# uthree/ALiVE-VC

Measured on AMD Instinct MI355X. Metric: VC frames/sec + RTF @24kHz, 1M-vec library; 1/2/4/8 MI355X, higher is better.
Workload: dtype decoder fp16 GEMMs / fp32 acc; encoders 22-bit fp16 split; kNN exact fp32 top-k via fp6 MFMA candidates (certified); f32 MFMA small convs; f64 phase scan

## Files before the change

### alive-vc_amd/csrc/knn.hip

```cpp
#include "common.h"

namespace {

constexpr int D = ALIVE_DIM;
constexpr int KP = ALIVE_KPRIME;
constexpr int TILE = 128;
constexpr int MAX_SPLIT = 64;

__device__ __forceinline__ float wave_sum(float v) {
#pragma unroll
    for (int o = 32; o > 0; o >>= 1) v += __shfl_xor(v, o);
    return v;
}

struct NormDiv {
    float n, y;
};
__device__ __forceinline__ NormDiv norm_div(float n) {
    float y = __builtin_amdgcn_rcpf(n);
    const float e = fmaf(-n, y, 1.0f);
    y = fmaf(e, y, y);
    return NormDiv{n, y};
}
__device__ __forceinline__ float div_by(float x, const NormDiv& d) {
// ... 339 lines not shown
    for (int i = 0; i < D / 256; ++i) xs[tid + 256 * i] = v[i];
    __syncthreads();
    if (tid < 4) {
        for (int d = tid; d < D; d += 4) ss = fmaf(xs[d], xs[d], ss);
        red[tid] = ss;
    }
    __syncthreads();
    const float nrm = sqrtf(red[0] + red[1] + red[2] + red[3]);
    if (nrm_out != nullptr && tid == 0) nrm_out[ft] = nrm;
    float e2 = 0.0f;
#pragma unroll
    for (int i = 0; i < D / 256; ++i) {
        const float q = nrm > 0.0f ? v[i] / nrm : 0.0f;
        s_f32[(size_t)ft * D + tid + 256 * i] = q;
        const unsigned short b = f32_to_bf16_rn(q);
        s_bf16[(size_t)ft * D + tid + 256 * i] = b;
        const float e = q - __uint_as_float((unsigned)b << 16);
        e2 = fmaf(e, e, e2);
    }
    if (dq != nullptr) {
        e2 = wave_sum(e2);
        if ((tid & 63) == 0) ered[tid >> 6] = e2;
        __syncthreads();
        if (tid == 0) dq[ft] = sqrtf(ered[0] + ered[1] + ered[2] + ered[3]) * 1.0001f;
    }
}

constexpr int KH = KP / 2;
constexpr int FT = 256;
constexpr int LT = 32;
constexpr int NK16 = D / 16;
constexpr int PIECE = 1152;
constexpr int NPIECE = 4 * (D / 64);
constexpr int ABUF = NPIECE * PIECE;
constexpr int SCORE_LDS = 2 * ABUF + FT * KP * 8;

constexpr int GATE_BOOL = -2;
__device__ __forceinline__ bool gate_open(const int* cnt, int lo, int hi, int& c) {
    c = 0x7fffffff;
    if (cnt == nullptr) return true;
    c = *cnt;
    return c > lo && c <= hi;
}

__global__ __launch_bounds__(128) void gather_frames_kernel(const unsigned short* __restrict__ s_bf16, const int* __restrict__ list,
                                                            const int* __restrict__ cnt, int lo, int hi, unsigned short* __restrict__ out) {
    int c;
    if (!gate_open(cnt, lo, hi, c)) return;
    const int slot = blockIdx.x;
    if (slot >= (c + 255) / 256 * 256) return;
    if (threadIdx.x >= 96) return;
    u32x4 v = {0u, 0u, 0u, 0u};
    if (slot < c) v = ((const u32x4*)(s_bf16 + (size_t)list[slot] * D))[threadIdx.x];
    ((u32x4*)(out + (size_t)slot * D))[threadIdx.x] = v;
}

typedef const __attribute__((address_space(1))) void* gptr_t;
typedef __attribute__((address_space(3))) void* lptr_t;

struct SeedArgs {
    float* tau;
    int* flag;
    int k;
    float margin;
    int* cnt;
};

__device__ __forceinline__ bool seeds_look(const SeedArgs& sa, int split) {
    __shared__ int verdict[1];
    if (sa.tau == nullptr || split == 0) return false;
    if (threadIdx.x == 0) {
        const int f = __hip_atomic_load(sa.flag + (size_t)(split - 1) * gridDim.x + blockIdx.x, __ATOMIC_RELAXED, __HIP_MEMORY_SCOPE_AGENT);
        if (f != 0) {
            atomicAdd(sa.cnt, 1);
            __builtin_amdgcn_fence(__ATOMIC_ACQUIRE, "agent");
        }
        verdict[0] = f;
    }
    asm volatile("s_waitcnt vmcnt(0)" ::: "memory");
    __syncthreads();
    return __builtin_amdgcn_readfirstlane(verdict[0]) != 0;
}

template <int KH_, int WF_ = 64, int FRAMES_ = 256>
__device__ __forceinline__ void seeds_publish(const SeedArgs& sa, const float* Lv, const int* Li, int64_t frame0, int split, bool seeded) {
    constexpr int LW_ = 4 * 2 * WF_;
    for (int col = threadIdx.x; col < FRAMES_; col += 256) {
        const int lcb = (col / WF_) * (2 * WF_) + ((col % WF_) >> 5) * 64 + (col & 31);
        float prev = INFINITY;
        for (int j = 0; j < sa.k; ++j) {
            float m = -INFINITY;
            for (int e = 0; e < 2 * KH_; ++e) {
                const int o = (e % KH_) * LW_ + lcb + (e / KH_) * 32;
                const float v = Lv[o];
                if (Li[o] >= 0 && v < prev) m = fmaxf(m, v);
            }
            prev = m;
        }
        float t = prev - sa.margin;
        if (seeded) {
            const float tin = sa.tau[frame0 + col];
            t = fmaxf(t, tin == tin ? tin : -INFINITY);
        }
        sa.tau[frame0 + col] = t;
    }
    asm volatile("s_waitcnt vmcnt(0)" ::: "memory");
    __syncthreads();
    if (threadIdx.x == 0) {
        __builtin_amdgcn_fence(__ATOMIC_RELEASE, "agent");
        asm volatile("s_waitcnt vmcnt(0)" ::: "memory");
        __hip_atomic_store(sa.flag + (size_t)split * gridDim.x + blockIdx.x, 1, __ATOMIC_RELAXED, __HIP_MEMORY_SCOPE_AGENT);
    }
}

struct PoolBlocks {
    const int* hdr;
    const int* blk_voice;
    const int64_t* img_off;
    const int32_t* seg_lo;
    const int32_t* seg_len;
};
enum { PH_GROUPS = 0, PH_BLOCKS, PH_ITEMS, PH_FAIL, PH_WORDS = 8 };

template <bool COLLECT, bool POOL = false>
__global__ __launch_bounds__(256, 1) void knn_score_kernel(const unsigned short* __restrict__ s_bf16,
                                                           const unsigned short* __restrict__ lib, int64_t M, int tiles_total,
                                                           int tiles_per_split, int P, float* __restrict__ cand_val,
                                                           int* __restrict__ cand_idx, const int* __restrict__ gate_cnt,
                                                           int gate_lo, int gate_hi, int by_count, const float* __restrict__ thr_in,
                                                           SeedArgs sa, int caps, PoolBlocks pool = PoolBlocks{}) {
    int n_slots = 0x7fffffff;
    {
        int c;
        if (!gate_open(gate_cnt, gate_lo, gate_hi, c)) return;
        if (by_count && (int64_t)blockIdx.x * 256 >= c) return;
        if (by_count) n_slots = c;
    }
    int row_base = 0;
    if constexpr (POOL) {
        if ((int)blockIdx.x >= pool.hdr[PH_BLOCKS]) return;
        const int v = pool.blk_voice[blockIdx.x];
        M = pool.seg_len[v];
        lib += (size_t)pool.img_off[v] * D;
        tiles_total = (int)(((M + TILE - 1) / TILE * TILE) / LT);
        tiles_per_split = (tiles_total + (int)gridDim.y - 1) / (int)gridDim.y;
        row_base = pool.seg_lo[v];
    }
    extern __shared__ __attribute__((aligned(16))) unsigned char smem[];
    float* Lv = (float*)(smem + 2 * ABUF);
    int* Li = (int*)(Lv + FT * KP);

    const int tid = threadIdx.x, lane = tid & 63;
    const int w = __builtin_amdgcn_readfirstlane(tid >> 6);
    const int lr = lane & 31, lh = lane >> 5;
    const int64_t frame0 = (int64_t)blockIdx.x * FT;
    const int split = blockIdx.y;
    const int tile_begin = split * tiles_per_split;
    int tile_end = tile_begin + tiles_per_split;
    if (tile_end > tiles_total) tile_end = tiles_total;

    const bool seeded = !COLLECT && seeds_look(sa, split);
    float seed[2] = {-INFINITY, -INFINITY};
    if (seeded) {
#pragma unroll
        for (int ni = 0; ni < 2; ++ni) {
            const float t = sa.tau[frame0 + 64 * w + 32 * ni + lr];
            seed[ni] = t == t ? t : -INFINITY;
        }
    }
    int* cntF = (int*)Lv;
    if (COLLECT) {
        cntF[tid] = 0;
        for (int e = tid; e < FT * caps; e += 256) {
            const size_t o = ((size_t)(frame0 + e / caps) * P + split) * caps + e % caps;
            cand_val[o] = -INFINITY;
            cand_idx[o] = -1;
        }
    } else {
// ... 275 lines not shown
            bf16x8 a[PD + 1];
#pragma unroll
            for (int i = 0; i < PD; ++i) a[i] = *(const bf16x8*)(Ab + a_off[i & 3] + (i >> 2) * 4 * PIECE);
#pragma unroll
            for (int ks = 0; ks < NK16; ++ks) {
                if (ks + PD < NK16) a[(ks + PD) % (PD + 1)] = *(const bf16x8*)(Ab + a_off[(ks + PD) & 3] + ((ks + PD) >> 2) * 4 * PIECE);
                if ((ks & 3) == 1)
                    __builtin_amdgcn_global_load_lds((gptr_t)(gnext + (ks >> 2) * 64), (lptr_t)(lnext + (ks >> 2) * 4 * PIECE), 16, 0, 0);
                __builtin_amdgcn_sched_barrier(0);
                acc = __builtin_amdgcn_mfma_f32_32x32x16_bf16(a[ks % (PD + 1)], bq[0][ks], acc, 0, 0, 0);
                __builtin_amdgcn_sched_barrier(0);
            }
        }
        const int64_t row0 = (int64_t)tile * LT;
        const bool ragged = row0 + LT > M;
        float mx = -INFINITY;
#pragma unroll
        for (int r = 0; r < 16; ++r) {
            if (ragged && row0 + (r & 3) + 8 * (r >> 2) + 4 * lh >= M) acc[r] = -INFINITY;
            mx = fmaxf(mx, acc[r]);
        }
        while (__builtin_amdgcn_ballot_w64(mx >= thr && mx > -INFINITY) != 0) {
            const bool has = mx >= thr && mx > -INFINITY;
            int rsel = 0;
#pragma unroll
            for (int r = 1; r < 16; ++r) rsel = (acc[r] == mx) ? r : rsel;
            if (has) {
                const int pos = atomicAdd(&cntF[32 * w + lr], 1);
                if (pos < caps) {
                    cand_val[seg + pos] = mx;
                    cand_idx[seg + pos] = (int)(row0 + (rsel & 3) + 8 * (rsel >> 2) + 4 * lh);
                }
            }
            float nmx = -INFINITY;
#pragma unroll
            for (int r = 0; r < 16; ++r) {
                if (has && r == rsel) acc[r] = -INFINITY;
                nmx = fmaxf(nmx, acc[r]);
            }
            mx = nmx;
        }
        __syncthreads();
    }
    if (tid < FT2 && cntF[tid] > caps) cand_idx[((size_t)(frame0 + tid) * P + split) * caps] = -2;
}

constexpr int KH8 = 16;
constexpr int KP8 = 2 * KH8;
constexpr int NK64 = D / 64;
constexpr int NPIECE8 = 4 * (D / 128);
constexpr int ABUF8 = NPIECE8 * PIECE;
constexpr int FT6 = 4 * 32 * 3;
constexpr int SCORE8_LDS = 2 * ABUF8 + FT * KP8 * 8;
constexpr int SCORE6_LDS = 2 * ABUF8 + FT6 * KP8 * 8;
typedef int v8i __attribute__((ext_vector_type(8)));

constexpr float SEED_MARGIN8 = 0.02f * F8_SCALE * F8_SCALE;
constexpr float SEED_MARGIN6 = 0.024f * F6_SCALE * F6_SCALE;
constexpr float SEED_MARGIN16 = 2.5e-3f;
constexpr float SEED_MARGIN16_STRICT = 4.5e-3f;
constexpr int SEED_MIN_FB = 512;
constexpr int SEED_MIN_FB6 = 300;

template <int FMT, int NCT8, int NK = NK64>
__device__ __forceinline__ void knn_score8_body(const unsigned char* __restrict__ s_f8,
                                                const unsigned char* __restrict__ lib, int64_t M, int tiles_total,
                                                int tiles_per_split, int P, float* __restrict__ cand_val,
                                                int* __restrict__ cand_idx, const int* __restrict__ gate_cnt,
                                                int gate_lo, int gate_hi, SeedArgs sa,
                                                const float* __restrict__ rho = nullptr, const float* __restrict__ gq = nullptr) {
    {
        int c;
        if (!gate_open(gate_cnt, gate_lo, gate_hi, c)) return;
    }
    constexpr int WF8 = 32 * NCT8;
    constexpr int FT8 = 4 * WF8;
    constexpr int LW8 = 4 * 2 * WF8;
    constexpr int KD = 64 * NK;
    constexpr int NSEG = KD / 128;
    constexpr int ABUF_ = 4 * NSEG * PIECE;
    extern __shared__ __attribute__((aligned(16))) unsigned char smem[];
    float* Lv = (float*)(smem + 2 * ABUF_);
    int* Li = (int*)(Lv + FT8 * KP8);

    const int tid = threadIdx.x, lane = tid & 63;
    const int w = __builtin_amdgcn_readfirstlane(tid >> 6);
    const int lr = lane & 31, lh = lane >> 5;
    const int64_t frame0 = (int64_t)blockIdx.x * FT8;
    const int split = blockIdx.y;
    const int tile_begin = split * tiles_per_split;
    int tile_end = tile_begin + tiles_per_split;
    if (tile_end > tiles_total) tile_end = tiles_total;

    const bool seeded = seeds_look(sa, split);
    float seed[NCT8];
#pragma unroll
    for (int ni = 0; ni < NCT8; ++ni) seed[ni] = -INFINITY;
    if (seeded) {
#pragma unroll
        for (int ni = 0; ni < NCT8; ++ni) {
            const float t = sa.tau[frame0 + WF8 * w + 32 * ni + lr];
            seed[ni] = t == t ? t : -INFINITY;
        }
    }
#pragma unroll
    for (int ni = 0; ni < NCT8; ++ni)
#pragma unroll
        for (int q = 0; q < KH8; ++q) { Lv[q * LW8 + w * (2 * WF8) + ni * 64 + lane] = seed[ni]; Li[q * LW8 + w * (2 * WF8) + ni * 64 + lane] = -1; }

    const int dma_row = 8 * w + (lane >> 3);
    const int dma_chunk = (lane & 7) ^ (lane >> 3);
    auto issue_tile = [&](int tile, int buf) {
        const unsigned char* g = lib + ((size_t)tile * LT + dma_row) * KD + dma_chunk * 16;
        unsigned char* l = smem + buf * ABUF_ + w * PIECE;
#pragma unroll
        for (int sg = 0; sg < NSEG; ++sg)
            __builtin_amdgcn_global_load_lds((gptr_t)(g + sg * 128), (lptr_t)(l + sg * 4 * PIECE), 16, 0, 0);
    };
    if (tile_begin < tile_end) issue_tile(tile_begin, 0);

    v8i bq[NCT8][NK];
#pragma unroll
    for (int ni = 0; ni < NCT8; ++ni) {
        const unsigned char* fp = s_f8 + (size_t)(frame0 + WF8 * w + 32 * ni + lr) * KD + 32 * lh;
#pragma unroll
        for (int ks = 0; ks < NK; ++ks) {
            if constexpr (FMT == 2) {
                const u32x4 lo = *(const u32x4*)(fp + 64 * ks);
                const uint2 hi = *(const uint2*)(fp + 64 * ks + 16);
                bq[ni][ks] = v8i{(int)lo[0], (int)lo[1], (int)lo[2], (int)lo[3], (int)hi.x, (int)hi.y, 0, 0};
            } else {
                const u32x4 lo = *(const u32x4*)(fp + 64 * ks), hi = *(const u32x4*)(fp + 64 * ks + 16);
                bq[ni][ks] = v8i{(int)lo[0], (int)lo[1], (int)lo[2], (int)lo[3], (int)hi[0], (int)hi[1], (int)hi[2], (int)hi[3]};
            }
        }
    }

    float gs[NCT8];
#pragma unroll
    for (int ni = 0; ni < NCT8; ++ni) gs[ni] = NK == NK64 ? 0.0f : gq[frame0 + WF8 * w + 32 * ni + lr] * (F6_SCALE * F6_SCALE);

    const int rr = lr & 7;
    int a_off[2][2];
#pragma unroll
    for (int j = 0; j < 2; ++j)
#pragma unroll
        for (int c = 0; c < 2; ++c) a_off[j][c] = (lr >> 3) * PIECE + rr * 128 + (((4 * j + 2 * lh + c) ^ rr) << 4);

    float qv[NCT8][4];
    int qp[NCT8][4];
#pragma unroll
    for (int ni = 0; ni < NCT8; ++ni)
#pragma unroll
        for (int q = 0; q < 4; ++q) { qv[ni][q] = seed[ni]; qp[ni][q] = 4 * q; }
    float thr[NCT8];
#pragma unroll
    for (int ni = 0; ni < NCT8; ++ni) thr[ni] = seed[ni];
    const int lc0 = w * (2 * WF8) + lane;
    __syncthreads();

    auto load_a = [&](const unsigned char* Ab, int ks) {
        const unsigned char* q = Ab + (ks >> 1) * 4 * PIECE;
        if constexpr (FMT == 2) {
            unsigned off0 = (unsigned)(uintptr_t)(lptr_t)(q + a_off[ks & 1][0]);
            const unsigned off1 = (unsigned)(uintptr_t)(lptr_t)(q + a_off[ks & 1][1]);
            uint2 h8;
            asm volatile("ds_read_b64 %0, %2" : "=v"(h8), "+v"(off0) : "v"(off1));
            const u32x4 lo = *(const __attribute__((address_space(3))) u32x4*)(uintptr_t)off0;
            return v8i{(int)lo[0], (int)lo[1], (int)lo[2], (int)lo[3], (int)h8.x, (int)h8.y, 0, 0};
        }
        const u32x4 lo = *(const u32x4*)(q + a_off[ks & 1][0]);
        const u32x4 hi = *(const u32x4*)(q + a_off[ks & 1][1]);
        return v8i{(int)lo[0], (int)lo[1], (int)lo[2], (int)lo[3], (int)hi[0], (int)hi[1], (int)hi[2], (int)hi[3]};
    };

    auto mask_ragged = [&](f32x16& acc, int tile) {
        const int64_t row0 = (int64_t)tile * LT;
        if (row0 + LT > M) {
            asm volatile("" ::: "memory");
            const int left = (int)(M - row0);
#pragma unroll
            for (int r = 0; r < 16; ++r)
                if (4 * lh >= left - ((r & 3) + 8 * (r >> 2))) acc[r] = -INFINITY;
        }
    };
    auto max8 = [&](const f32x16& acc, int lo, float m) {
#pragma unroll
        for (int r = 0; r < 8; ++r) m = fmaxf(m, acc[lo + r]);
        return m;
    };
    auto load_rho = [&](int tile, float* rv) {
#pragma unroll
        for (int j = 0; j < 4; ++j) {
            const f32x4 t = *(const f32x4*)(rho + (size_t)tile * LT + 8 * j + 4 * lh);
#pragma unroll
            for (int e = 0; e < 4; ++e) rv[4 * j + e] = t[e];
        }
    };
    auto max8g = [&](f32x16& acc, int lo, float m, int ni, const float* rv) {
#pragma unroll
        for (int r = 0; r < 8; ++r) acc[lo + r] = fmaf(gs[ni], rv[lo + r], acc[lo + r]);
        return max8(acc, lo, m);
    };
    auto fold_loop = [&](f32x16& acc, int ni, int tile, float mx) {
        const int64_t row0 = (int64_t)tile * LT;
        float* lv = Lv + lc0 + ni * 64;
        int* li = Li + lc0 + ni * 64;
        while (__builtin_amdgcn_ballot_w64(mx > thr[ni]) != 0) {
            const bool has = mx > thr[ni];
            const bool b01 = qv[ni][1] < qv[ni][0], b23 = qv[ni][3] < qv[ni][2];
            const float m01 = b01 ? qv[ni][1] : qv[ni][0], m23 = b23 ? qv[ni][3] : qv[ni][2];
            const int p01 = b01 ? qp[ni][1] : qp[ni][0], p23 = b23 ? qp[ni][3] : qp[ni][2];
            const bool bq = m23 < m01;
            const int tpos = bq ? p23 : p01;
            const int tq = tpos >> 2;
            if (has) {
                lv[tpos * LW8] = mx;
                li[tpos * LW8] = (int)(row0 + ((__float_as_uint(mx) & 3u) + 8u * ((__float_as_uint(mx) >> 2) & 3u)) + 4 * lh);
            }
            const float* qb = lv + (tq * 4) * LW8;
            const float x0 = qb[0], x1 = qb[LW8], x2 = qb[2 * LW8], x3 = qb[3 * LW8];
            const bool c1 = x1 < x0, c3 = x3 < x2;
            const float n01 = c1 ? x1 : x0, n23 = c3 ? x3 : x2;
            const int e01 = c1 ? 1 : 0, e23 = c3 ? 3 : 2;
            const bool c = n23 < n01;
            const float nq = c ? n23 : n01;
            const int np = tq * 4 + (c ? e23 : e01);
#pragma unroll
            for (int q = 0; q < 4; ++q) {
                const bool hit = has && tq == q;
                qv[ni][q] = hit ? nq : qv[ni][q];
                qp[ni][q] = hit ? np : qp[ni][q];
            }
            thr[ni] = fminf(fminf(qv[ni][0], qv[ni][1]), fminf(qv[ni][2], qv[ni][3]));
            float nmx = -INFINITY;
#pragma unroll
            for (int r = 0; r < 16; ++r) nmx = fmaxf(nmx, acc[r] < mx ? acc[r] : -INFINITY);
            mx = has ? nmx : mx;
        }
    };

    auto fold_rare = [&](f32x16& acc, int ni, int tile, float mx) {
        if (__builtin_amdgcn_ballot_w64(mx > thr[ni]) == 0) return;
        const int64_t row0 = (int64_t)tile * LT;
        float* lv = Lv + lc0 + ni * 64;
        int* li = Li + lc0 + ni * 64;
        const bool b01 = qv[ni][1] < qv[ni][0], b23 = qv[ni][3] < qv[ni][2];
        const float m01 = b01 ? qv[ni][1] : qv[ni][0], m23 = b23 ? qv[ni][3] : qv[ni][2];
        const int p01 = b01 ? qp[ni][1] : qp[ni][0], p23 = b23 ? qp[ni][3] : qp[ni][2];
        const int tpos = m23 < m01 ? p23 : p01;
        const int tq = tpos >> 2, te = tpos & 3;
        const float* qb = lv + (tq * 4) * LW8;
        float x0 = qb[0], x1 = qb[LW8], x2 = qb[2 * LW8], x3 = qb[3 * LW8];
#pragma unroll
        for (int r = 0; r < 16; ++r) acc[r] = __uint_as_float((__float_as_uint(acc[r]) & ~15u) | (unsigned)r);
        if (row0 + LT > M) {
            asm volatile("" ::: "memory");
            const int left = (int)(M - row0);
#pragma unroll
            for (int r = 0; r < 16; ++r)
                if (4 * lh >= left - ((r & 3) + 8 * (r >> 2))) acc[r] = -INFINITY;
        }
        float m1 = -INFINITY, m2 = -INFINITY;
#pragma unroll
        for (int r = 0; r < 16; ++r) {
            m2 = __builtin_amdgcn_fmed3f(m1, m2, acc[r]);
            m1 = fmaxf(m1, acc[r]);
        }
        const bool has = m1 > thr[ni];
        if (has) {
            const unsigned u = __float_as_uint(m1);
            lv[tpos * LW8] = m1;
            li[tpos * LW8] = (int)(row0 + ((u & 3u) + 8u * ((u >> 2) & 3u)) + 4 * lh);
        }
        x0 = (has && te == 0) ? m1 : x0;
        x1 = (has && te == 1) ? m1 : x1;
        x2 = (has && te == 2) ? m1 : x2;
        x3 = (has && te == 3) ? m1 : x3;
        const bool c1 = x1 < x0, c3 = x3 < x2;
        const float n01 = c1 ? x1 : x0, n23 = c3 ? x3 : x2;
        const int e01 = c1 ? 1 : 0, e23 = c3 ? 3 : 2;
        const bool c = n23 < n01;
        const float nq = c ? n23 : n01;
        const int np = tq * 4 + (c ? e23 : e01);
#pragma unroll
        for (int q = 0; q < 4; ++q) {
            const bool hit = has && tq == q;
            qv[ni][q] = hit ? nq : qv[ni][q];
            qp[ni][q] = hit ? np : qp[ni][q];
        }
        thr[ni] = fminf(fminf(qv[ni][0], qv[ni][1]), fminf(qv[ni][2], qv[ni][3]));
        fold_loop(acc, ni, tile, m2);
    };
    if constexpr (NCT8 == 3) {
    auto do_tile3 = [&](int tile, f32x16& c0, f32x16& c1, f32x16& c2, f32x16& p0, f32x16& p1, f32x16& p2, float* rv, float* rn) {
        const int buf = (tile - tile_begin) & 1;
        const int next_tile = tile + 1 < tile_end ? tile + 1 : tile;
        const unsigned char* gnext = lib + ((size_t)next_tile * LT + dma_row) * KD + dma_chunk * 16;
        unsigned char* lnext = smem + (buf ^ 1) * ABUF_ + w * PIECE;
        const unsigned char* Ab = smem + buf * ABUF_;
#pragma unroll
        for (int r = 0; r < 16; ++r) { c0[r] = 0.0f; c1[r] = 0.0f; c2[r] = 0.0f; }
        if constexpr (NK != NK64) load_rho(tile, rn);
        constexpr int PD6 = 1, NA6 = PD6 + 1;
        v8i a[NA6];
#pragma unroll
        for (int i = 0; i < PD6; ++i) a[i] = load_a(Ab, i);
        float pm0 = -INFINITY, pm1 = -INFINITY, pm2 = -INFINITY;
        ALIVE_CHAIN_GAP(7);
#define K8_STEP3(ks, AFTER0, AFTER1, AFTER2)                                                                                     \
        {                                                                                                                        \
            __builtin_amdgcn_sched_barrier(0);                                                                                   \
            c0 = __builtin_amdgcn_mfma_scale_f32_32x32x64_f8f6f4(a[(ks) % NA6], bq[0][ks], c0, FMT, FMT, 0, 127, 0, 127); \
            __builtin_amdgcn_sched_barrier(0);                                                                                   \
            if ((ks) + PD6 < NK) a[((ks) + PD6) % NA6] = load_a(Ab, (ks) + PD6);                                                 \
            if ((ks) < NSEG)                                                                                                     \
                __builtin_amdgcn_global_load_lds((gptr_t)(gnext + (ks) * 128), (lptr_t)(lnext + (ks) * 4 * PIECE), 16, 0, 0);    \
            AFTER0;                                                                                                              \
            __builtin_amdgcn_sched_barrier(0);                                                                                   \
            c1 = __builtin_amdgcn_mfma_scale_f32_32x32x64_f8f6f4(a[(ks) % NA6], bq[1][ks], c1, FMT, FMT, 0, 127, 0, 127); \
            __builtin_amdgcn_sched_barrier(0);                                                                                   \
            AFTER1;                                                                                                              \
            __builtin_amdgcn_sched_barrier(0);                                                                                   \
            c2 = __builtin_amdgcn_mfma_scale_f32_32x32x64_f8f6f4(a[(ks) % NA6], bq[2][ks], c2, FMT, FMT, 0, 127, 0, 127); \
            __builtin_amdgcn_sched_barrier(0);                                                                                   \
            AFTER2;                                                                                                              \
        }
        f32x16 v0, v1, v2;
        auto acc_read = [&](const f32x16& a_, int lo, int hi, f32x16& v) {
#pragma unroll
            for (int r = lo; r < hi; ++r) asm volatile("v_accvgpr_read_b32 %0, %1" : "=v"(v[r]) : "a"(a_[r]));
        };
        auto acc_pin = [&]() { asm volatile("" : "+a"(c0), "+a"(c1), "+a"(c2)); };
        K8_STEP3(0, (void)0, (void)0, (void)0) K8_STEP3(1, (void)0, (void)0, (void)0) K8_STEP3(2, (void)0, (void)0, (void)0)
        if constexpr (NK == NK64) {
        K8_STEP3(3, (void)0, (void)0, (void)0) K8_STEP3(4, (void)0, (void)0, (void)0) K8_STEP3(5, (void)0, (void)0, acc_pin())
        }
        if constexpr (NK == NK64) {
        K8_STEP3(6, acc_read(p0, 0, 8, v0), (acc_pin(), acc_read(p0, 8, 16, v0), mask_ragged(v0, tile - 1)), (acc_pin(), pm0 = max8(v0, 0, pm0)))
        K8_STEP3(7, pm0 = max8(v0, 8, pm0), fold_rare(v0, 0, tile - 1, pm0), (acc_pin(), acc_read(p1, 0, 8, v1)))
        K8_STEP3(8, (acc_pin(), acc_read(p1, 8, 16, v1), mask_ragged(v1, tile - 1)), (acc_pin(), pm1 = max8(v1, 0, pm1)), pm1 = max8(v1, 8, pm1))
        K8_STEP3(9, fold_rare(v1, 1, tile - 1, pm1), (acc_pin(), acc_read(p2, 0, 8, v2)), (acc_pin(), acc_read(p2, 8, 16, v2), mask_ragged(v2, tile - 1)))
        K8_STEP3(10, (acc_pin(), pm2 = max8(v2, 0, pm2)), pm2 = max8(v2, 8, pm2), fold_rare(v2, 2, tile - 1, pm2))
        K8_STEP3(11, (void)0, (void)0, (void)0)
        } else {
        K8_STEP3(3, acc_pin(), (acc_pin(), acc_read(p0, 0, 8, v0)), (acc_pin(), acc_read(p0, 8, 16, v0), mask_ragged(v0, tile - 1)))
        K8_STEP3(4, (acc_pin(), pm0 = max8g(v0, 0, pm0, 0, rv)), pm0 = max8g(v0, 8, pm0, 0, rv), fold_rare(v0, 0, tile - 1, pm0))
        K8_STEP3(5, (acc_pin(), acc_read(p1, 0, 8, v1)), (acc_pin(), acc_read(p1, 8, 16, v1), mask_ragged(v1, tile - 1)), (acc_pin(), pm1 = max8g(v1, 0, pm1, 1, rv)))
        K8_STEP3(6, pm1 = max8g(v1, 8, pm1, 1, rv), fold_rare(v1, 1, tile - 1, pm1), (acc_pin(), acc_read(p2, 0, 8, v2)))
        K8_STEP3(7, (acc_pin(), acc_read(p2, 8, 16, v2), mask_ragged(v2, tile - 1)), (acc_pin(), pm2 = max8g(v2, 0, pm2, 2, rv)),
                 (pm2 = max8g(v2, 8, pm2, 2, rv), fold_rare(v2, 2, tile - 1, pm2)))
        }
#undef K8_STEP3
        acc_pin();
        __syncthreads();
    };
    auto fold_now3 = [&](f32x16& p0, f32x16& p1, f32x16& p2, int tile, float* rv) {
        mask_ragged(p0, tile);
        mask_ragged(p1, tile);
        mask_ragged(p2, tile);
        if constexpr (NK != NK64) {
            (void)max8g(p0, 0, max8g(p0, 8, -INFINITY, 0, rv), 0, rv);
            (void)max8g(p1, 0, max8g(p1, 8, -INFINITY, 1, rv), 1, rv);
            (void)max8g(p2, 0, max8g(p2, 8, -INFINITY, 2, rv), 2, rv);
        }
        fold_rare(p0, 0, tile, max8(p0, 8, max8(p0, 0, -INFINITY)));
        fold_rare(p1, 1, tile, max8(p1, 8, max8(p1, 0, -INFINITY)));
        fold_rare(p2, 2, tile, max8(p2, 8, max8(p2, 0, -INFINITY)));
    };
    {
        f32x16 A0, A1, A2, B0, B1, B2;
        float RA[16], RB[16];
#pragma unroll
        for (int r = 0; r < 16; ++r) { B0[r] = -INFINITY; B1[r] = -INFINITY; B2[r] = -INFINITY; RA[r] = 0.0f; RB[r] = 0.0f; }
        int tile = tile_begin;
        for (; tile + 1 < tile_end; tile += 2) {
            do_tile3(tile, A0, A1, A2, B0, B1, B2, RB, RA);
            do_tile3(tile + 1, B0, B1, B2, A0, A1, A2, RA, RB);
        }
        if (tile < tile_end) {
            do_tile3(tile, A0, A1, A2, B0, B1, B2, RB, RA);
            fold_now3(A0, A1, A2, tile, RA);
        } else if (tile_begin < tile_end) {
            fold_now3(B0, B1, B2, tile_end - 1, RB);
        }
    }
    } else {
    auto do_tile = [&](int tile, f32x16& c0, f32x16& c1, f32x16& p0, f32x16& p1) {
        const int buf = (tile - tile_begin) & 1;
        const int next_tile = tile + 1 < tile_end ? tile + 1 : tile;
        const unsigned char* gnext = lib + ((size_t)next_tile * LT + dma_row) * KD + dma_chunk * 16;
        unsigned char* lnext = smem + (buf ^ 1) * ABUF_ + w * PIECE;
        const unsigned char* Ab = smem + buf * ABUF_;
#pragma unroll
        for (int r = 0; r < 16; ++r) { c0[r] = 0.0f; c1[r] = 0.0f; }
        v8i a[2];
        a[0] = load_a(Ab, 0);
        float pm0 = -INFINITY, pm1 = -INFINITY;
#ifndef ALIVE_KNN8_NO_CHAIN_GAP
        ALIVE_CHAIN_GAP(7);
#endif
#define K8_STEP(ks, AFTER0, AFTER1)                                                                                              \
        {                                                                                                                        \
            __builtin_amdgcn_sched_barrier(0);                                                                                   \
            c0 = __builtin_amdgcn_mfma_scale_f32_32x32x64_f8f6f4(a[(ks) & 1], bq[0][ks], c0, FMT, FMT, 0, 127, 0, 127);              \
            __builtin_amdgcn_sched_barrier(0);                                                                                   \
            if ((ks) + 1 < NK) a[((ks) + 1) & 1] = load_a(Ab, (ks) + 1);                                                         \
            if ((ks) < NSEG)      \
                                 \
                __builtin_amdgcn_global_load_lds((gptr_t)(gnext + (ks) * 128), (lptr_t)(lnext + (ks) * 4 * PIECE), 16, 0, 0);    \
            AFTER0;                                                                                                              \
            __builtin_amdgcn_sched_barrier(0);                                                                                   \
            c1 = __builtin_amdgcn_mfma_scale_f32_32x32x64_f8f6f4(a[(ks) & 1], bq[1][ks], c1, FMT, FMT, 0, 127, 0, 127);              \
            __builtin_amdgcn_sched_barrier(0);                                                                                   \
            AFTER1;                                                                                                              \
        }
        f32x16 v0, v1;
        auto acc_read = [&](const f32x16& a, int lo, int hi, f32x16& v) {
#pragma unroll
            for (int r = lo; r < hi; ++r) asm volatile("v_accvgpr_read_b32 %0, %1" : "=v"(v[r]) : "a"(a[r]));
        };
        auto acc_pin = [&]() { asm volatile("" : "+a"(c0), "+a"(c1)); };
        K8_STEP(0, (void)0, (void)0) K8_STEP(1, (void)0, (void)0) K8_STEP(2, (void)0, (void)0) K8_STEP(3, (void)0, (void)0)
        K8_STEP(4, (void)0, (void)0) K8_STEP(5, (void)0, acc_pin())
        K8_STEP(6, acc_read(p0, 0, 8, v0), (acc_pin(), acc_read(p0, 8, 16, v0), mask_ragged(v0, tile - 1)))
        K8_STEP(7, (acc_pin(), pm0 = max8(v0, 0, pm0)), pm0 = max8(v0, 8, pm0))
        K8_STEP(8, (acc_pin(), acc_read(p1, 0, 8, v1)), (acc_pin(), acc_read(p1, 8, 16, v1), mask_ragged(v1, tile - 1)))
        K8_STEP(9, (acc_pin(), pm1 = max8(v1, 0, pm1)), pm1 = max8(v1, 8, pm1))
        K8_STEP(10, (void)0, fold_rare(v0, 0, tile - 1, pm0))
        K8_STEP(11, (void)0, fold_rare(v1, 1, tile - 1, pm1))
#undef K8_STEP
        asm volatile("" : "+a"(c0), "+a"(c1));
        __syncthreads();
    };
    auto fold_now = [&](f32x16& p0, f32x16& p1, int tile) {
        mask_ragged(p0, tile);
        mask_ragged(p1, tile);
        fold_rare(p0, 0, tile, max8(p0, 8, max8(p0, 0, -INFINITY)));
        fold_rare(p1, 1, tile, max8(p1, 8, max8(p1, 0, -INFINITY)));
    };

    f32x16 A0, A1, B0, B1;
#pragma unroll
    for (int r = 0; r < 16; ++r) { B0[r] = -INFINITY; B1[r] = -INFINITY; }
    int tile = tile_begin;
    for (; tile + 1 < tile_end; tile += 2) {
        do_tile(tile, A0, A1, B0, B1);
        do_tile(tile + 1, B0, B1, A0, A1);
    }
    if (tile < tile_end) {
        do_tile(tile, A0, A1, B0, B1);
        fold_now(A0, A1, tile);
    } else if (tile_begin < tile_end) {
        fold_now(B0, B1, tile_end - 1);
    }
    }
    __syncthreads();

    for (int e = tid; e < FT8 * KP8; e += 256) {
        const int k = e % KP8, col = e / KP8;
        const int lc = (col / WF8) * (2 * WF8) + ((col % WF8) >> 5) * 64 + (k / KH8) * 32 + (col & 31);
        const size_t o = (((size_t)(frame0 + col)) * P + split) * KP8 + k;
        cand_val[o] = Lv[(k % KH8) * LW8 + lc];
        cand_idx[o] = Li[(k % KH8) * LW8 + lc];
    }
    if (sa.tau != nullptr) seeds_publish<KH8, WF8, FT8>(sa, Lv, Li, frame0, split, seeded);
}

__global__ __launch_bounds__(256, 1) void knn_score8_kernel(const unsigned char* __restrict__ s_f8, const unsigned char* __restrict__ lib,
                                                            int64_t M, int tiles_total, int tiles_per_split, int P,
                                                            float* __restrict__ cand_val, int* __restrict__ cand_idx,
                                                            const int* __restrict__ gate_cnt, int gate_lo, int gate_hi, SeedArgs sa) {
    knn_score8_body<0, 2>(s_f8, lib, M, tiles_total, tiles_per_split, P, cand_val, cand_idx, gate_cnt, gate_lo, gate_hi, sa);
}
__global__ __launch_bounds__(256, 1) void knn_probe8_kernel(const unsigned char* __restrict__ s_f8, const unsigned char* __restrict__ lib,
                                                            int64_t M, int tiles_total, int tiles_per_split, int P,
                                                            float* __restrict__ cand_val, int* __restrict__ cand_idx, const int* __restrict__ gate) {
    knn_score8_body<0, 2>(s_f8, lib, M, tiles_total, tiles_per_split, P, cand_val, cand_idx, gate, 0, 1, SeedArgs{nullptr, nullptr, 0, 0.0f, nullptr});
}
__global__ __launch_bounds__(256, 1) void knn_score6_kernel(const unsigned char* __restrict__ s_f6, const unsigned char* __restrict__ lib,
                                                            int64_t M, int tiles_total, int tiles_per_split, int P,
                                                            float* __restrict__ cand_val, int* __restrict__ cand_idx,
                                                            const int* __restrict__ gate_cnt, int gate_lo, int gate_hi, SeedArgs sa) {
    knn_score8_body<2, 3>(s_f6, lib, M, tiles_total, tiles_per_split, P, cand_val, cand_idx, gate_cnt, gate_lo, gate_hi, sa);
}
__global__ __launch_bounds__(256, 1) void knn_probe6_kernel(const unsigned char* __restrict__ s_f6, const unsigned char* __restrict__ lib,
                                                            int64_t M, int tiles_total, int tiles_per_split, int P,
                                                            float* __restrict__ cand_val, int* __restrict__ cand_idx, const int* __restrict__ gate) {
    knn_score8_body<2, 3>(s_f6, lib, M, tiles_total, tiles_per_split, P, cand_val, cand_idx, gate, 0, 1, SeedArgs{nullptr, nullptr, 0, 0.0f, nullptr});
}
constexpr int NK_SUB = 8;
constexpr int SUB_K = 64 * NK_SUB;
constexpr int SUB6_LDS = 2 * 4 * (SUB_K / 128) * PIECE + FT6 * KP8 * 8;
__global__ __launch_bounds__(256, 1) void knn_sub6_kernel(const unsigned char* __restrict__ s_sub, const unsigned char* __restrict__ lib_sub,
                                                          const float* __restrict__ rho, const float* __restrict__ gq,
                                                          int64_t M, int tiles_total, int tiles_per_split, int P,
                                                          float* __restrict__ cand_val, int* __restrict__ cand_idx,
                                                          const int* __restrict__ gate_cnt, int gate_lo, int gate_hi, SeedArgs sa) {
    knn_score8_body<2, 3, NK_SUB>(s_sub, lib_sub, M, tiles_total, tiles_per_split, P, cand_val, cand_idx, gate_cnt, gate_lo, gate_hi, sa,
                                  rho, gq);
}

template <int G>
__device__ __forceinline__ float wave_sum_frames(float (&d)[G], int lane) {
    if constexpr (G >= 16) {
        const bool up = lane & 32;
#pragma unroll
        for (int j = 0; j < 8; ++j) d[j] = (up ? d[8 + j] : d[j]) + __shfl_xor(up ? d[j] : d[8 + j], 32);
    }
    if constexpr (G >= 8) {
        constexpr int o = G >= 16 ? 16 : 32;
        const bool up = lane & o;
#pragma unroll
        for (int j = 0; j < 4; ++j) d[j] = (up ? d[4 + j] : d[j]) + __shfl_xor(up ? d[j] : d[4 + j], o);
    }
    if constexpr (G >= 4) {
        constexpr int o = G >= 16 ? 8 : (G >= 8 ? 16 : 32);
        const bool up = lane & o;
#pragma unroll
        for (int j = 0; j < 2; ++j) d[j] = (up ? d[2 + j] : d[j]) + __shfl_xor(up ? d[j] : d[2 + j], o);
    }
    if constexpr (G >= 2) {
        constexpr int o = G >= 16 ? 4 : (G >= 8 ? 8 : (G >= 4 ? 16 : 32));
        const bool up = lane & o;
        d[0] = (up ? d[1] : d[0]) + __shfl_xor(up ? d[0] : d[1], o);
    }
    float v = d[0];
#pragma unroll
    for (int o = 32 / G; o > 0; o >>= 1) v += __shfl_xor(v, o);
    return v;
}

__device__ __forceinline__ int wave_argbest(float v, int idx) {
    float bv = v;
    int bi = idx;
    int bl = threadIdx.x & 63;
#pragma unroll
    for (int o = 32; o > 0; o >>= 1) {
        float ov = __shfl_xor(bv, o);
        int oi = __shfl_xor(bi, o);
        int ol = __shfl_xor(bl, o);
        bool take = (ov > bv) || (ov == bv && (unsigned)oi < (unsigned)bi) || (ov == bv && oi == bi && ol < bl);
        if (take) { bv = ov; bi = oi; bl = ol; }
    }
    return bl;
}

struct PoolRescore {
    const int* slot_grp;
    const int* grp;
    int* gfail;
    int* fb;
};
enum { PG_VOICE = 0, PG_MSTART, PG_SIZE, PG_BLK0, PG_NBLK, PG_CHUNKS, PG_NSLAB, PG_BASE, PG_FBASE, PG_K, PG_FIELDS };

template <int PER, bool POOL = false, bool HAT = false>
__global__ __launch_bounds__(256) __attribute__((amdgpu_waves_per_eu(HAT && PER < 16 ? 8 : 1))) void knn_rescore_kernel(const float* __restrict__ cand_val, const int* __restrict__ cand_idx,
                                                          int P, int kp, const float* __restrict__ s_f32,
                                                          const float* __restrict__ rows, const float* __restrict__ norms,
                                                          const float* __restrict__ rows_hat,
                                                          int64_t Tt, int64_t idx_base, int k, float* __restrict__ out_val,
                                                          int* __restrict__ out_idx, const int* __restrict__ frame_list,
                                                          const int* __restrict__ gate_cnt, int gate_lo, int gate_hi,
                                                          int* __restrict__ flag_list, int* __restrict__ flag_cnt, float zsig,
                                                          int list_len, float pre_scale, float sd_prior,
                                                          const float* __restrict__ det_q, const float* __restrict__ det_lib,
                                                          float* __restrict__ thr_list, int collect, float overflow_slack,
                                                          const unsigned char* __restrict__ force_fail = nullptr,
                                                          PoolRescore pool = PoolRescore{}) {
    __shared__ float cs_v[4][64];
    __shared__ int cs_i[4][64];
    const int lane = threadIdx.x & 63, wv = threadIdx.x >> 6;
    const int64_t slot = (int64_t)blockIdx.x * 4 + wv;
    int gc;
    if (gate_lo == GATE_BOOL) {
        if (*gate_cnt == 0) return;
        gc = 0x7fffffff;
    } else if (!gate_open(gate_cnt, gate_lo, gate_hi, gc)) {
        return;
    }
    if (slot >= Tt || (frame_list != nullptr && slot >= gc)) return;
    const int64_t ft = frame_list != nullptr ? frame_list[slot] : slot;
// ... 897 lines not shown
            const float up_v = __shfl_up(lv, 1);
            const int up_i = __shfl_up(li, 1);
            const bool up_before = (lane % k == 0) ? true : (up_v > p || (up_v == p && up_i < (int)r));
            if (live && !before) {
                lv = up_before ? p : up_v;
                li = up_before ? (int)r : up_i;
            }
            if (G < 16) {
                q0 = n0; q1 = n1; q2 = n2; nn = nnn;
            } else if (r + nw < M) {
                const f32x4* rp = (const f32x4*)(rows + (size_t)(r + nw) * D);
                q0 = rp[lane]; q1 = rp[lane + 64]; q2 = rp[lane + 128];
                nn = norms[r + nw];
            }
        }
        part_val[(size_t)item * 64 + lane] = lv;
        part_idx[(size_t)item * 64 + lane] = li;
    }
}

template <int G>
__global__ __launch_bounds__(256) void knn_exact_merge_kernel(const float* __restrict__ part_val, const int* __restrict__ part_idx,
                                                              int64_t Tt, int k, int64_t idx_base, const int* __restrict__ frame_list,
                                                              const int* __restrict__ cnt_ptr, float* __restrict__ out_val,
                                                              int* __restrict__ out_idx, int max_count) {
    __shared__ float sv[256];
    __shared__ int si[256], sw[256];
    const int tid = threadIdx.x;
    int64_t count = Tt;
    if (cnt_ptr != nullptr) { const int c = *cnt_ptr; count = c < Tt ? c : Tt; }
    if (count > max_count) return;
    const int64_t groups = (count + G - 1) / G;
    const int nw = exact_nw(groups);
    constexpr int NL = EX_NW_MAX / 256;
    for (int64_t slot = blockIdx.x; slot < count; slot += gridDim.x) {
        const int64_t g = slot / G;
        const int t = (int)(slot - g * G);
        const int64_t ft = frame_list != nullptr ? frame_list[slot] : slot;
        int head[NL];
#pragma unroll
        for (int i = 0; i < NL; ++i) head[i] = 0;
        for (int j = 0; j < k; ++j) {
            float bv = -INFINITY;
            int bi = 0x7fffffff, bl = -1;
#pragma unroll
            for (int i = 0; i < NL; ++i) {
                const int w = tid + 256 * i;
                if (w < nw && head[i] < k) {
                    const size_t o = ((size_t)g * nw + w) * 64 + t * k + head[i];
                    const float v = part_val[o];
                    const int id = part_idx[o];
                    if (v > bv || (v == bv && id < bi)) { bv = v; bi = id; bl = i; }
                }
            }
            sv[tid] = bv; si[tid] = bi; sw[tid] = tid;
            __syncthreads();
            for (int o = 128; o > 0; o >>= 1) {
                if (tid < o) {
                    const float ov = sv[tid + o];
                    const int oi = si[tid + o];
                    if (ov > sv[tid] || (ov == sv[tid] && oi < si[tid])) { sv[tid] = ov; si[tid] = oi; sw[tid] = sw[tid + o]; }
                }
                __syncthreads();
            }
            if (tid == 0) {
                out_val[(size_t)ft * k + j] = sv[0];
                out_idx[(size_t)ft * k + j] = (si[0] == 0x7fffffff || !(sv[0] > -INFINITY)) ? -1 : (int)(idx_base + si[0]);
            }
            if (sw[0] == tid && bl >= 0) {
#pragma unroll
                for (int i = 0; i < NL; ++i)
                    if (i == bl) head[i]++;
            }
            __syncthreads();
        }
    }
}

constexpr int COLLECT_MIN = 256;
constexpr int RESEARCH_MIN = 64;
enum { ST_FLAG8 = 0, ST_FLAG16 = 1, ST_PROBE_N = 2, ST_PROBE_FAIL = 3, ST_MODE = 4, ST_FIRST = 5, ST_PROBE_CNT = 6, ST_TIER = 7, ST_FLAGC = 8, ST_SEEDED = 9, ST_SEEDED16 = 10, ST_RESEARCH_MIN = 11, ST_COLLECT_MIN = 12,
       ST_PROBE_SKIPPED = 13,
       ST_SUB_FLAG = 14, ST_SUB_CLIP = 15, ST_SUB_FORM = 20, ST_SUB_GATE = 21,
       ST_HIST_TAG = 16, ST_HIST_STREAK = 17, ST_HIST_CALLS = 18, ST_PROBE_GATE = 19,
       ST_WORDS = 32 };
constexpr int PROBE_EVERY = 16, PROBE_STREAK = 2;
enum { TIER_SCAN = 1, TIER_EXACT_ALL = 2, TIER_BF16 = 3, TIER_FP8 = 4, TIER_FP6 = 5 };
__device__ __forceinline__ bool fp6_slot(const float* v, u32x4* o) {
    unsigned long long acc = 0;
    int nb = 0, wi = 0;
    unsigned wd[6];
    bool clipped = false;
#pragma unroll
    for (int j = 0; j < 32; ++j) {
        clipped = clipped || fabsf(v[j]) > 7.75f;
        acc |= (unsigned long long)fp6_e2m3(v[j]) << nb;
        nb += 6;
        if (nb >= 32) { wd[wi++] = (unsigned)acc; acc >>= 32; nb -= 32; }
    }
    o[0] = u32x4{wd[0], wd[1], wd[2], wd[3]};
    o[1] = u32x4{wd[4], wd[5], 0u, 0u};
    return clipped;
}
constexpr int SUB_C = 576;
__global__ __launch_bounds__(256) void lib_sub6_kernel(const float* __restrict__ y, int64_t count, int64_t span, unsigned char* __restrict__ out,
                                                       float* __restrict__ rho, int* __restrict__ clip) {
    const int64_t i = (int64_t)blockIdx.x * 256 + threadIdx.x;
    if (i >= span * (SUB_K / 32)) return;
    const int64_t r = i / (SUB_K / 32);
    const int grp = (int)(i % (SUB_K / 32));
    float v[32];
#pragma unroll
    for (int j = 0; j < 32; ++j) v[j] = r < count ? y[(size_t)r * SUB_C + 32 * grp + j] * F6_SCALE : 0.0f;
    if (fp6_slot(v, (u32x4*)(out + (size_t)r * SUB_K + 32 * grp))) atomicOr(clip, 1);
    if (grp == 0) rho[r] = r < count ? y[(size_t)r * SUB_C + SUB_K] : 0.0f;
}
constexpr float SUB_RES2 = 1.0e-5f;
__global__ __launch_bounds__(256) void sub_codes_kernel(const float* __restrict__ y, const float* __restrict__ nrm, int T, int64_t Tt,
                                                        int64_t Tt_pad, unsigned char* __restrict__ out, float* __restrict__ g,
                                                        unsigned char* __restrict__ flag, int* __restrict__ stats) {
    __shared__ float ssq[8][32];
    __shared__ int clp[8][32];
    const int fl = threadIdx.x & 31, cg = threadIdx.x >> 5;
    const int64_t f = (int64_t)blockIdx.x * 32 + fl;
    const bool live = f < Tt;
    const int64_t ni = live ? f / T : 0, ti = live ? f - ni * T : 0;
    const float* yb = y + (size_t)ni * SUB_C * T + ti;
    const float q = live ? nrm[f] : 0.0f;
    const float inv = q > 0.0f ? 1.0f / q : 0.0f;
    float v[32];
    float sy = 0.0f;
    bool clipped = false;
#pragma unroll
    for (int h = 0; h < 2; ++h) {
#pragma unroll
        for (int j = 0; j < 32; ++j) {
            v[j] = live ? yb[(size_t)(32 * (cg + 8 * h) + j) * T] * inv : 0.0f;
            sy = fmaf(v[j], v[j], sy);
            v[j] *= F6_SCALE;
        }
        u32x4 o[2];
        clipped = fp6_slot(v, o) || clipped;
        if (f < Tt_pad) {
            u32x4* dst = (u32x4*)(out + (size_t)f * SUB_K + 32 * (cg + 8 * h));
            dst[0] = o[0];
            dst[1] = o[1];
        }
    }
    const float gy = live ? yb[(size_t)SUB_K * T] * inv : 0.0f;
    if (cg == 0) sy = fmaf(gy, gy, sy);
    ssq[cg][fl] = sy;
    clp[cg][fl] = clipped ? 1 : 0;
    __syncthreads();
    if (cg == 0 && f < Tt_pad) {
        float s2 = 0.0f;
        int cl = 0;
#pragma unroll
        for (int k = 0; k < 8; ++k) { s2 += ssq[k][fl]; cl |= clp[k][fl]; }
        const bool out_of_span = q > 0.0f && 1.0f - s2 > SUB_RES2;
        const bool bad = live && (cl != 0 || out_of_span);
        g[f] = gy;
        flag[f] = bad ? 1 : 0;
        if (bad) atomicAdd(stats + ST_SUB_FLAG, 1);
        if (live && cl != 0) atomicAdd(stats + ST_SUB_CLIP, 1);
    }
}
__global__ __launch_bounds__(256) void sub_select_kernel(const unsigned char* __restrict__ flag, unsigned char* __restrict__ clip6,
                                                         int64_t n, int* __restrict__ stats) {
    const bool sub = stats[ST_SUB_FLAG] <= RESEARCH_MIN;
    const int64_t i = (int64_t)blockIdx.x * 256 + threadIdx.x;
    if (sub && i < n && flag[i] != 0) clip6[i] = 1;
    if (i == 0) {
        stats[ST_SUB_FORM] = sub ? 1 : 2;
        stats[ST_SUB_GATE] = stats[ST_MODE] != 0 ? 0 : (sub ? 1 : 2);
    }
}

__global__ void stats_init_kernel(int* __restrict__ stats, int tier, int hist_tag = 0) {
    if (threadIdx.x < ST_HIST_TAG)
        stats[threadIdx.x] = threadIdx.x == ST_TIER ? tier
                           : threadIdx.x == ST_RESEARCH_MIN ? RESEARCH_MIN : threadIdx.x == ST_COLLECT_MIN ? COLLECT_MIN : 0;
    if (threadIdx.x == ST_HIST_TAG) {
        const bool valid = hist_tag != 0 && stats[ST_HIST_TAG] == hist_tag;
        const int streak = valid ? stats[ST_HIST_STREAK] : 0, calls = valid ? stats[ST_HIST_CALLS] : 0;
        const bool skip = streak >= PROBE_STREAK && (calls % PROBE_EVERY) != 0;
        stats[ST_HIST_TAG] = hist_tag;
        stats[ST_HIST_STREAK] = streak;
        stats[ST_HIST_CALLS] = calls + 1;
        stats[ST_PROBE_GATE] = skip ? 0 : 1;
        stats[ST_PROBE_SKIPPED] = skip ? 1 : 0;
    }
}
__global__ void probe_history_kernel(int* __restrict__ stats, int64_t Tt) {
    const bool clean = stats[ST_MODE] == 0 && (int64_t)stats[ST_FLAG8] * 20 <= Tt &&
                       (stats[ST_PROBE_GATE] == 0 || (int64_t)stats[ST_PROBE_FAIL] * 4 <= (int64_t)stats[ST_PROBE_N]);
    stats[ST_HIST_STREAK] = clean ? stats[ST_HIST_STREAK] + 1 : 0;
}
__global__ __launch_bounds__(64) void probe_gather_kernel(const unsigned char* __restrict__ s_f8, int64_t Tt, int n, int n_pad,
                                                          unsigned char* __restrict__ out, int* __restrict__ plist, const int* __restrict__ gate) {
    if (*gate == 0) return;
    const int slot = blockIdx.x;
    if (slot >= n_pad) return;
    u32x4 v = {0u, 0u, 0u, 0u};
    if (slot < n) {
        const int64_t ft = (int64_t)slot * Tt / n;
        if (threadIdx.x < D / 16) v = ((const u32x4*)(s_f8 + (size_t)ft * D))[threadIdx.x];
        if (threadIdx.x == 0) plist[slot] = (int)ft;
    }
    if (threadIdx.x < D / 16) ((u32x4*)(out + (size_t)slot * D))[threadIdx.x] = v;
}

__global__ void probe_decide_kernel(int* __restrict__ stats, int n, int num, int den) {
    if (stats[ST_PROBE_GATE] == 0) return;
    const int fail = stats[ST_PROBE_CNT];
    stats[ST_PROBE_N] = n;
    stats[ST_PROBE_FAIL] = fail;
    stats[ST_MODE] = ((int64_t)fail * den > (int64_t)n * num) ? 1 : 0;
}

__global__ __launch_bounds__(256) void flag_all_kernel(int* __restrict__ list, int* __restrict__ cnt, int64_t Tt,
                                                       const int* __restrict__ gate_cnt, int gate_lo, int gate_hi) {
    int c;
    if (!gate_open(gate_cnt, gate_lo, gate_hi, c)) return;
    const int64_t i = (int64_t)blockIdx.x * 256 + threadIdx.x;
    if (i < Tt) list[i] = (int)i;
    if (i == 0) *cnt = (int)Tt;
}

__global__ __launch_bounds__(256) void dedup_pass_kernel(const float* __restrict__ val, const int* __restrict__ idx, int64_t M, int k,
                                                         float threshold, int* __restrict__ state, int* __restrict__ undecided) {
    const int64_t i = (int64_t)blockIdx.x * 256 + threadIdx.x;
    if (i >= M || state[i] != 0) return;
    bool any_kept = false, all_dropped = true;
    for (int q = 0; q < k; ++q) {
        const int j = idx[i * k + q];
        if (j < 0 || j >= i || !(val[i * k + q] > threshold)) continue;
        const int sj = ((volatile int*)state)[j];
        any_kept |= sj == 1;
        all_dropped &= sj == 2;
    }
    if (any_kept) state[i] = 2;
    else if (all_dropped) state[i] = 1;
    else atomicAdd(undecided, 1);
}


struct SearchPlan {
    int64_t Tt, Tt_pad;
    int tiles_total, split, tiles_per_split, P;
};

static SearchPlan make_plan(int64_t Tt, int64_t M, int split_cap = MAX_SPLIT, int ft = FT) {
    SearchPlan p;
    p.Tt = Tt;
    p.Tt_pad = (Tt + ft - 1) / ft * ft;
    p.tiles_total = (int)(((M + TILE - 1) / TILE * TILE) / LT);
    const int64_t fb = p.Tt_pad / ft;
    int max_split = p.tiles_total / 8;
    if (max_split > split_cap) max_split = split_cap;
    if (max_split < 1) max_split = 1;
    int best = 1;
    double best_eff = -1.0;
    auto eff_of = [&](int sp) {
        const int64_t blocks = fb * sp, rounds = (blocks + 255) / 256;
        return (double)blocks / (double)(rounds * 256);
    };
    for (int sp = 1; sp <= max_split; ++sp) {
        const double eff = eff_of(sp);
        if (eff > best_eff + 0.02) { best_eff = eff; best = sp; }
    }
    if (ft != FT) {
        double top = 0.0;
        for (int sp = 1; sp <= max_split; ++sp) top = eff_of(sp) > top ? eff_of(sp) : top;
        for (int sp = 1; sp <= max_split; ++sp)
            if (eff_of(sp) >= top - 0.03) { best = sp; break; }
    }
    p.split = best;
    p.tiles_per_split = (p.tiles_total + best - 1) / best;
    p.P = best;
    return p;
}

constexpr int MAX_SPLIT8 = 1024 / KP8;
constexpr int FCAP = 16384;
constexpr int TIER1A = 256;
constexpr int FPLAN = 4096;
constexpr float CERT_Z = 7.0f;
constexpr float SD_PRIOR6 = 2.0e-3f;
constexpr float SD_PRIOR8R = 2.5e-4f;
constexpr float SD_PRIOR8 = 1.5e-3f;
constexpr float SD_PRIOR16 = 8.0e-5f;
constexpr int PROBE_N = 1024;
constexpr int64_t PROBE_MIN_T = 16384;
constexpr int PROBE_NUM = 11, PROBE_DEN = 20;

static SeedArgs seeds_for(const struct SearchWs& w, int64_t fb, int split, int k, float margin, int counter, hipStream_t s, int min_fb = SEED_MIN_FB);

struct SearchWs {
    SearchPlan p16, p8, pt, pp;
    SearchPlan p6, pp6;
    SearchPlan pa;
    int fcap, probe_n, probe_pad, probe_pad6;
    float* s_f32; unsigned short* s_bf16; unsigned char* s_f8;
    float* cv; int* ci;
    float* pv; int* pi;
    int* stats; int* list0; int* list1;
    unsigned short* s_c;
    float* cv1; int* ci1;
    unsigned char* s_p8; float* cvp; int* cip; int* p_list;
    float* thr1; int* list2;
    float* dq;
    unsigned char* clip6;
    unsigned char* sub_f6; float* sub_g; unsigned char* sub_flag;
    float* sub_nrm;
    unsigned short* sub_planes; float* sub_y;
    unsigned short* s_c2h; unsigned short* s_c2l;
    float* c2v; int* c2i;
    int rows_t, rows_b;
    const unsigned short* lib_lo;
    float* tau; int* tau_flag;
    const float* det_q; const float* det_lib;
    const float* rows_hat;
    size_t bytes;
};

static SearchWs ws_layout(void* base, int64_t Tt, int64_t M, int k, bool split = false, bool sub = false) {
    SearchWs w;
    w.p16 = make_plan(Tt, M);
    w.p8 = make_plan(Tt, M, MAX_SPLIT8);
    w.p6 = make_plan(Tt, M, MAX_SPLIT8, FT6);
    const int64_t Tp = w.p16.Tt_pad;
    const int64_t Tp8 = w.p6.Tt_pad > Tp ? w.p6.Tt_pad : Tp;
    w.fcap = Tp < FCAP ? (int)Tp : FCAP;
    w.pt = make_plan(w.fcap < FPLAN ? w.fcap : FPLAN, M);
    w.pa = make_plan(FT, M);
    w.probe_n = Tt >= PROBE_MIN_T ? PROBE_N : 0;
    w.probe_pad = (w.probe_n + FT - 1) / FT * FT;
    w.probe_pad6 = (w.probe_n + FT6 - 1) / FT6 * FT6;
    w.pp = make_plan(w.probe_n > 0 ? w.probe_n : 1, M, MAX_SPLIT8);
    w.pp6 = make_plan(w.probe_n > 0 ? w.probe_n : 1, M, MAX_SPLIT8, FT6);
    Arena a(base);
    w.stats = a.take<int>(ST_WORDS);
    w.s_f32 = a.take<float>((size_t)Tt * D);
    w.s_bf16 = a.take<unsigned short>((size_t)Tp * D);
    w.s_f8 = a.take<unsigned char>((size_t)Tp8 * D);
    const size_t c8a = (size_t)Tp * w.p8.P * KP8, c8b = (size_t)w.p6.Tt_pad * w.p6.P * KP8;
    const size_t c16 = (size_t)Tp * w.p16.P * KP, c8 = c8a > c8b ? c8a : c8b;
    w.cv = a.take<float>(c16 > c8 ? c16 : c8);
    w.ci = a.take<int>(c16 > c8 ? c16 : c8);
    size_t lists = exact_lists(Tt, k <= ALIVE_MAX_K && k >= 1 ? k : 4);
    if (lists < (size_t)SCAN_MAX_LISTS) lists = SCAN_MAX_LISTS;
    w.pv = a.take<float>(lists * 64);
    w.pi = a.take<int>(lists * 64);
    w.list0 = a.take<int>((size_t)Tp);
    w.list1 = a.take<int>((size_t)Tp);
    w.s_c = a.take<unsigned short>((size_t)Tp * D);
    const size_t n1a = (size_t)(w.fcap < TIER1A ? w.fcap : TIER1A) * w.pa.P * KP, n1 = (size_t)w.fcap * w.pt.P * KP;
    w.cv1 = a.take<float>(n1 > n1a ? n1 : n1a);
    w.ci1 = a.take<int>(n1 > n1a ? n1 : n1a);
    const size_t ppad = w.probe_pad6 > w.probe_pad ? w.probe_pad6 : w.probe_pad;
    const size_t pcand = ppad * (size_t)(w.pp6.P > w.pp.P ? w.pp6.P : w.pp.P) * KP8;
    w.s_p8 = a.take<unsigned char>(ppad * D + 16);
    w.cvp = a.take<float>(pcand + 4);
    w.cip = a.take<int>(pcand + 4);
    w.p_list = a.take<int>(2 * ppad + 8);
    w.thr1 = a.take<float>((size_t)Tp);
    w.list2 = a.take<int>((size_t)Tp);
    w.dq = a.take<float>((size_t)Tp);
    w.clip6 = a.take<unsigned char>((size_t)Tp8);
    const size_t c2n = (size_t)(Tp < FCAP ? Tp : FCAP) * 1024 > (size_t)Tp * SPLIT_ROWS ? (size_t)(Tp < FCAP ? Tp : FCAP) * 1024 : (size_t)Tp * SPLIT_ROWS;
    w.c2v = a.take<float>(c2n);
    w.c2i = a.take<int>(c2n);
    w.rows_t = (int)(c2n / (size_t)w.fcap < 1024 ? c2n / (size_t)w.fcap : 1024);
    w.rows_b = (int)(c2n / (size_t)Tp < 1024 ? c2n / (size_t)Tp : 1024);
    w.lib_lo = nullptr;
    w.tau = a.take<float>((size_t)Tp8);
    w.tau_flag = a.take<int>((size_t)(Tp / FT) * (MAX_SPLIT > MAX_SPLIT8 ? MAX_SPLIT : MAX_SPLIT8));
    w.det_q = nullptr;
    w.det_lib = nullptr;
    w.rows_hat = nullptr;
    w.s_c2h = split ? a.take<unsigned short>((size_t)Tp * D) : nullptr;
    w.s_c2l = split ? a.take<unsigned short>((size_t)Tp * D) : nullptr;
    w.sub_f6 = sub ? a.take<unsigned char>((size_t)Tp8 * SUB_K) : nullptr;
    w.sub_g = sub ? a.take<float>((size_t)Tp8) : nullptr;
    w.sub_nrm = sub ? a.take<float>((size_t)Tp8) : nullptr;
    w.sub_flag = sub ? a.take<unsigned char>((size_t)Tp8) : nullptr;
    w.sub_planes = sub ? a.take<unsigned short>(alive_planes_bytes(Tt, D, 2) / 2) : nullptr;
    w.sub_y = sub ? a.take<float>((size_t)Tt * SUB_C) : nullptr;
    w.bytes = a.used() + 1024;
    return w;
}

static SeedArgs seeds_for(const SearchWs& w, int64_t fb, int split, int k, float margin, int counter, hipStream_t s, int min_fb) {
    if (fb < min_fb || split < 2) return SeedArgs{nullptr, nullptr, 0, 0.0f, nullptr};
    (void)hipMemsetAsync(w.tau_flag, 0, (size_t)fb * split * sizeof(int), s);
    return SeedArgs{w.tau, w.tau_flag, k, margin, w.stats + counter};
}


constexpr int POOL_MAX_ROWS = 4096;
constexpr int POOL_MAX_FRAMES = 1 << 20;
constexpr int POOL_MERGE_BLOCKS = 1024;

struct PoolWs {
    int* stats;
    int* hdr;
    float* s_f32; unsigned short* s_bf16; float* dq;
    unsigned short* s_c;
    float* cv; int* ci;
    int* slot_frame; int* slot_grp;
    int* grp;
    int* members;
    int* blk_voice; int* blk_grp;
    int* gfail;
    int* fb;
    float* pv; int* pi;
    int64_t S;
    int P;
    int64_t items;
    size_t bytes;
};

static PoolWs pool_ws_layout(void* base, int N, int T, int k, int V, int64_t max_len, int kinds = 1) {
    PoolWs w{};
    const int64_t Tt = (int64_t)N * T;
    const int64_t gmax = N < (int64_t)V * kinds ? N : (int64_t)V * kinds;
    w.S = ((Tt + FT - 1) / FT + gmax) * FT;
    w.P = make_plan(Tt, max_len).split;
    const int F = 64 / k;
    const int64_t chunks = (Tt + F - 1) / F + gmax;
    w.items = chunks > GR_ITEMS ? chunks : GR_ITEMS;
    Arena a(base);
    w.stats = a.take<int>(ALIVE_POOL_STATS);
    w.hdr = a.take<int>(PH_WORDS);
    w.s_f32 = a.take<float>((size_t)Tt * D);
    w.s_bf16 = a.take<unsigned short>((size_t)((Tt + 63) / 64 * 64) * D);
    w.dq = a.take<float>((size_t)Tt);
    w.s_c = a.take<unsigned short>((size_t)w.S * D);
    w.cv = a.take<float>((size_t)w.S * w.P * KP);
    w.ci = a.take<int>((size_t)w.S * w.P * KP);
    w.slot_frame = a.take<int>((size_t)w.S);
    w.slot_grp = a.take<int>((size_t)w.S);
    w.grp = a.take<int>((size_t)(N + 1) * PG_FIELDS);
    w.members = a.take<int>((size_t)N);
    w.blk_voice = a.take<int>((size_t)(w.S / FT));
    w.blk_grp = a.take<int>((size_t)(w.S / FT));
    w.gfail = a.take<int>((size_t)N);
    w.fb = a.take<int>((size_t)w.S);
    w.pv = a.take<float>((size_t)w.items * 64);
    w.pi = a.take<int>((size_t)w.items * 64);
    w.bytes = a.used();
    return w;
}

__global__ __launch_bounds__(256) void pool_image_kernel(const float* __restrict__ rows, const float* __restrict__ norms, int64_t M,
                                                         int64_t M_pad, unsigned short* __restrict__ lib) {
    const int64_t i = (int64_t)blockIdx.x * 256 + threadIdx.x;
    if (i >= M_pad * D) return;
    const int64_t m = i / D;
    const float q = m < M ? rows[i] / norms[m] : 0.0f;
// ... 219 lines not shown
        const int g = pool_group_of(w.grp, G, PG_FBASE, i);
        const int* e = w.grp + g * PG_FIELDS;
        const int kg = MODE == MERGE_ROW ? e[PG_K] : k, F = 64 / kg;
        const int pos = i - e[PG_FBASE];
        const int c = pos / F;
        const int ft = w.slot_frame[w.fb[(int64_t)e[PG_BLK0] * FT + pos]];
        const size_t off = (size_t)(e[PG_BASE] + c) * 64;
        if constexpr (MODE == MERGE_ROW) {
            if (kg <= 4) scan_merge_frame<true>(w.pv + off, w.pi + off, (int64_t)e[PG_CHUNKS] * 64, e[PG_NSLAB], pos - c * F, kg, 0, out_val, out_idx, ft, k);
            else scan_merge_frame<false>(w.pv + off, w.pi + off, (int64_t)e[PG_CHUNKS] * 64, e[PG_NSLAB], pos - c * F, kg, 0, out_val, out_idx, ft, k);
        } else {
            scan_merge_frame<MODE == MERGE_K4>(w.pv + off, w.pi + off, (int64_t)e[PG_CHUNKS] * 64, e[PG_NSLAB], pos - c * F, kg, 0, out_val, out_idx, ft, k);
        }
        __syncthreads();
    }
}

}

extern "C" int64_t alive_library_padded_rows(int64_t M) { return (M + TILE - 1) / TILE * TILE; }

extern "C" int alive_library_pack(const float* tokens, int64_t M, int Dd, void* lib_bf16, float* rows_f32, float* norms,
                                  void* stream) {
    ALIVE_CHECK_ARG(tokens && lib_bf16 && rows_f32 && norms, "alive_library_pack: null pointer");
    ALIVE_CHECK_ARG(Dd == D, "alive_library_pack: feature dim %d, expected %d", Dd, D);
    ALIVE_CHECK_ARG(M >= 1 && M < (int64_t)1 << 31, "alive_library_pack: M out of range");
    int64_t M_pad = alive_library_padded_rows(M);
    lib_pack_kernel<<<(unsigned)(M_pad / 64), 256, 0, (hipStream_t)stream>>>(tokens, M, M_pad, (unsigned short*)lib_bf16,
                                                                            rows_f32, norms);
    ALIVE_CHECK_LAUNCH("alive_library_pack");
    return ALIVE_OK;
}

static int knn_scan_launch(const float* src, int T, int64_t Tt, const float* rows_f32, const float* norms, int64_t M,
                           int64_t idx_base, int k, float* s_f32, unsigned short* s_bf16, float* pv, int* pi, float* out_val,
                           int32_t* out_idx, int* stats, hipStream_t s, hipEvent_t g_ev_start, hipEvent_t g_ev_stop) {
    stats_init_kernel<<<1, 64, 0, s>>>(stats, TIER_SCAN);
    src_prep_small_kernel<<<(unsigned)Tt, 256, 0, s>>>(src, T, Tt, s_f32, s_bf16, nullptr);
    int blocks = (int)((M + 4 * SCAN_WAVES - 1) / (4 * SCAN_WAVES));
    if (blocks > SCAN_MAX_LISTS / SCAN_WAVES) blocks = SCAN_MAX_LISTS / SCAN_WAVES;
    if (blocks < 1) blocks = 1;
    if (g_ev_start) (void)hipEventRecord(g_ev_start, s);
    knn_scan_kernel<true><<<blocks, 64 * SCAN_WAVES, 0, s>>>(s_f32, rows_f32, norms, M, (int)Tt, k, pv, pi);
    if (g_ev_stop) (void)hipEventRecord(g_ev_stop, s);
    if (k <= 4) knn_scan_merge_kernel<true><<<(unsigned)Tt, 256, 0, s>>>(pv, pi, blocks * SCAN_WAVES, k, idx_base, out_val, out_idx);
    else knn_scan_merge_kernel<false><<<(unsigned)Tt, 256, 0, s>>>(pv, pi, blocks * SCAN_WAVES, k, idx_base, out_val, out_idx);
    ALIVE_CHECK_LAUNCH("alive_knn_search(scan)");
    return ALIVE_OK;
}

static void knn_exact_launch(const SearchWs& w, const float* rows_f32, const float* norms, int64_t M, int64_t Tt, int64_t idx_base,
                             int k, const int* list, const int* cnt, float* out_val, int32_t* out_idx, hipStream_t s,
                             int max_count = 0x7fffffff) {
#define ALIVE_EXACT(G_)                                                                                                        \
    {                                                                                                                          \
        knn_exact_kernel<G_><<<EX_BLOCKS, 256, 0, s>>>(w.s_f32, rows_f32, norms, M, Tt, k, list, cnt, w.pv, w.pi, max_count);   \
        knn_exact_merge_kernel<G_><<<1024, 256, 0, s>>>(w.pv, w.pi, Tt, k, idx_base, list, cnt, out_val, out_idx, max_count);  \
    }
    switch (exact_group(k)) {
        case 16: ALIVE_EXACT(16) break;
        case 8: ALIVE_EXACT(8) break;
        case 4: ALIVE_EXACT(4) break;
        case 2: ALIVE_EXACT(2) break;
        default: ALIVE_EXACT(1) break;
    }
#undef ALIVE_EXACT
}

static void src_prep_launch(const SearchWs& w, const float* src, int T, int64_t Tt, hipStream_t s) {
    float* dq = w.det_q != nullptr ? w.dq : nullptr;
    if (Tt <= 512) src_prep_small_kernel<<<(unsigned)w.p16.Tt_pad, 256, 0, s>>>(src, T, Tt, w.s_f32, w.s_bf16, dq, w.sub_nrm);
    else src_prep_kernel<<<(unsigned)(w.p16.Tt_pad / 64), 256, 0, s>>>(src, T, Tt, w.p16.Tt_pad, w.s_f32, w.s_bf16, dq, w.sub_nrm);
}

static int check_search_args(const char* what, const void* a, const void* b, int N, int T, int k, int64_t M) {
    ALIVE_CHECK_ARG(a && b, "%s: null pointer", what);
    ALIVE_CHECK_ARG(N > 0 && T > 0, "%s: empty source", what);
    ALIVE_CHECK_ARG(k >= 1 && k <= ALIVE_MAX_K, "%s: k=%d outside [1,%d]", what, k, ALIVE_MAX_K);
    ALIVE_CHECK_ARG(M >= k, "%s: library shard has %lld vectors, fewer than k=%d", what, (long long)M, k);
    ALIVE_CHECK_ARG((int64_t)N * T < ((int64_t)1 << 31) - FT6, "%s: %lld frames in one call", what, (long long)N * T);
    return ALIVE_OK;
}

static int lds_optin(const char* what) {
    static LdsOptIn optin8, optin6, optin16, optin_split, optin_sub;
    hipError_t e = optin8.ensure({(const void*)knn_score8_kernel, (const void*)knn_probe8_kernel}, SCORE8_LDS);
    if (e == hipSuccess) e = optin6.ensure({(const void*)knn_score6_kernel, (const void*)knn_probe6_kernel}, SCORE6_LDS);
    if (e == hipSuccess) e = optin16.ensure({(const void*)knn_score_kernel<false>, (const void*)knn_score_kernel<true>}, SCORE_LDS);
    if (e == hipSuccess) e = optin_split.ensure({(const void*)knn_collect_split_kernel}, SPLIT_LDS);
    if (e == hipSuccess) e = optin_sub.ensure({(const void*)knn_sub6_kernel}, SUB6_LDS);
    if (e != hipSuccess) {
        alive_set_error("%s: cannot reserve %d B of LDS: %s", what, SCORE_LDS, hipGetErrorString(e));
        return ALIVE_ERR_LAUNCH;
    }
    return ALIVE_OK;
}

extern "C" size_t alive_library_fp8_bytes(int64_t M) { return (size_t)alive_library_padded_rows(M) * D; }

extern "C" int alive_library_pack_fp8(const void* lib_bf16, int64_t M, void* lib_f8, void* stream) {
    ALIVE_CHECK_ARG(lib_bf16 && lib_f8 && M >= 1, "alive_library_pack_fp8: bad args");
    const int64_t n8 = alive_library_padded_rows(M) * D / 8;
    lib_to_fp8_kernel<<<(unsigned)((n8 + 255) / 256), 256, 0, (hipStream_t)stream>>>((const unsigned short*)lib_bf16, n8, (uint2*)lib_f8);
    ALIVE_CHECK_LAUNCH("alive_library_pack_fp8");
    return ALIVE_OK;
}

extern "C" int alive_library_pack_fp6(const void* lib_bf16, int64_t M, void* lib_f6, void* stream) {
    ALIVE_CHECK_ARG(lib_bf16 && lib_f6 && M >= 1, "alive_library_pack_fp6: bad args");
    const int64_t n32 = alive_library_padded_rows(M) * D / 32;
    to_fp6_kernel<<<(unsigned)((n32 + 255) / 256), 256, 0, (hipStream_t)stream>>>((const unsigned short*)lib_bf16, n32, n32, (u32x4*)lib_f6);
    ALIVE_CHECK_LAUNCH("alive_library_pack_fp6");
    return ALIVE_OK;
}

extern "C" size_t alive_knn_workspace_bytes_fast(int64_t Tt, int64_t M) {
    const size_t a = ws_layout(nullptr, Tt, M, 4).bytes, b = ws_layout(nullptr, Tt, M, ALIVE_MAX_K).bytes;
    return a > b ? a : b;
}
extern "C" size_t alive_knn_workspace_bytes_strict(int64_t Tt, int64_t M) {
    const size_t a = ws_layout(nullptr, Tt, M, 4, true).bytes, b = ws_layout(nullptr, Tt, M, ALIVE_MAX_K, true).bytes;
    return a > b ? a : b;
}
extern "C" size_t alive_knn_workspace_bytes(int64_t Tt, int64_t M) { return alive_knn_workspace_bytes_strict(Tt, M); }
extern "C" size_t alive_knn_workspace_bytes_sub(int64_t Tt, int64_t M) {
    const size_t a = ws_layout(nullptr, Tt, M, 4, false, true).bytes, b = ws_layout(nullptr, Tt, M, ALIVE_MAX_K, false, true).bytes;
    return a > b ? a : b;
}

static void collect_tier_launch(const SearchWs& w, const void* lib_bf16, const float* rows_f32, const float* norms, int64_t M,
                                int64_t Tt, int64_t idx_base, int k, float* out_val, int32_t* out_idx, hipStream_t s) {
    int* cnt1 = w.stats + ST_FLAG16;
    int* cnt2 = w.stats + ST_FLAGC;
    const int fcap = w.fcap;
    if (w.lib_lo != nullptr) {
        const unsigned Tp = (unsigned)w.p16.Tt_pad;
        knn_exact_launch(w, rows_f32, norms, M, Tt, idx_base, k, w.list1, cnt1, out_val, out_idx, s, COLLECT_MIN);
        gather_frames_split_kernel<<<Tp, 128, 0, s>>>(w.s_bf16, w.s_f32, w.list1, cnt1, COLLECT_MIN, w.s_c2h, w.s_c2l);
        const int caps = w.rows_b / w.p16.P < 64 ? w.rows_b / w.p16.P : 64;
        knn_collect_split_kernel<<<dim3(Tp / FT2, w.p16.split), 256, SPLIT_LDS, s>>>(
            w.s_c2h, w.s_c2l, (const unsigned short*)lib_bf16, w.lib_lo, M, w.p16.tiles_total, w.p16.tiles_per_split, w.p16.P, caps,
            w.c2v, w.c2i, cnt1, COLLECT_MIN, w.thr1);
        rescore_launch((unsigned)((Tt + 3) / 4), s, w.c2v, w.c2i, w.p16.P, caps, w.s_f32, rows_f32, norms, w.rows_hat, Tt, idx_base, k,
                                                                   out_val, out_idx, w.list1, cnt1, COLLECT_MIN, 0x7fffffff, w.list2, cnt2,
                                                                   CERT_Z, KH, 1.0f, SD_PRIOR16, nullptr, nullptr, nullptr, 1, 0.0f);
        knn_exact_launch(w, rows_f32, norms, M, Tt, idx_base, k, w.list2, cnt2, out_val, out_idx, s);
        return;
    }
    const int caps_t = w.rows_t / w.pt.P < 64 ? w.rows_t / w.pt.P : 64, caps_b = w.rows_b / w.p16.P < 64 ? w.rows_b / w.p16.P : 64;
    knn_exact_launch(w, rows_f32, norms, M, Tt, idx_base, k, w.list1, cnt1, out_val, out_idx, s, COLLECT_MIN);
    gather_frames_kernel<<<(unsigned)fcap, 128, 0, s>>>(w.s_bf16, w.list1, cnt1, COLLECT_MIN, fcap, w.s_c);
    knn_score_kernel<true><<<dim3((unsigned)(fcap / FT), w.pt.split), 256, SCORE_LDS, s>>>(
        w.s_c, (const unsigned short*)lib_bf16, M, w.pt.tiles_total, w.pt.tiles_per_split, w.pt.P, w.c2v, w.c2i, cnt1, COLLECT_MIN, fcap, 1,
        w.thr1, SeedArgs{nullptr, nullptr, 0, 0.0f, nullptr}, caps_t);
    rescore_launch((unsigned)((fcap + 3) / 4), s, w.c2v, w.c2i, w.pt.P, caps_t, w.s_f32, rows_f32, norms, w.rows_hat, fcap, idx_base, k,
                                                                 out_val, out_idx, w.list1, cnt1, COLLECT_MIN, fcap, w.list2, cnt2, CERT_Z,
                                                                 KH, 1.0f, SD_PRIOR16, nullptr, nullptr, nullptr, 1, 0.0f);
    if (w.p16.Tt_pad > fcap) {
        gather_frames_kernel<<<(unsigned)w.p16.Tt_pad, 128, 0, s>>>(w.s_bf16, w.list1, cnt1, fcap, 0x7fffffff, w.s_c);
        knn_score_kernel<true><<<dim3((unsigned)(w.p16.Tt_pad / FT), w.p16.split), 256, SCORE_LDS, s>>>(
            w.s_c, (const unsigned short*)lib_bf16, M, w.p16.tiles_total, w.p16.tiles_per_split, w.p16.P, w.c2v, w.c2i, cnt1, fcap,
            0x7fffffff, 1, w.thr1, SeedArgs{nullptr, nullptr, 0, 0.0f, nullptr}, caps_b);
        rescore_launch((unsigned)((Tt + 3) / 4), s, w.c2v, w.c2i, w.p16.P, caps_b, w.s_f32, rows_f32, norms, w.rows_hat, Tt, idx_base, k,
                                                                   out_val, out_idx, w.list1, cnt1, fcap, 0x7fffffff, w.list2, cnt2,
                                                                   CERT_Z, KH, 1.0f, SD_PRIOR16, nullptr, nullptr, nullptr, 1, 0.0f);
    }
    knn_exact_launch(w, rows_f32, norms, M, Tt, idx_base, k, w.list2, cnt2, out_val, out_idx, s);
}

static void bf16_tiers_launch(const SearchWs& w, const void* lib_bf16, const float* rows_f32, const float* norms, int64_t M,
                              int64_t Tt, int64_t idx_base, int k, float* out_val, int32_t* out_idx, hipStream_t s) {
    int* cnt0 = w.stats + ST_FLAG8;
    int* cnt1 = w.stats + ST_FLAG16;
// ... 42 lines not shown
    }
    hipStream_t s = (hipStream_t)stream;
    if (Tt * k <= 64 && M <= SCAN_ROWS_MAX)
        return knn_scan_launch(src, T, Tt, rows_f32, norms, M, idx_base, k, w.s_f32, w.s_bf16, w.pv, w.pi, out_val, out_idx, w.stats, s, g_ev_start, g_ev_stop);
    if (int rc = lds_optin("alive_knn_search")) return rc;
    stats_init_kernel<<<1, 64, 0, s>>>(w.stats, k > KH ? TIER_EXACT_ALL : TIER_BF16);
    src_prep_launch(w, src, T, Tt, s);
    if (k > KH) {
        if (g_ev_start) (void)hipEventRecord(g_ev_start, s);
        knn_exact_launch(w, rows_f32, norms, M, Tt, idx_base, k, nullptr, nullptr, out_val, out_idx, s);
        if (g_ev_stop) (void)hipEventRecord(g_ev_stop, s);
        ALIVE_CHECK_LAUNCH("alive_knn_search(exact)");
        return ALIVE_OK;
    }
    const SearchPlan& p = w.p16;
    const SeedArgs sa = seeds_for(w, p.Tt_pad / FT, p.split, k, w.det_q != nullptr ? SEED_MARGIN16_STRICT : SEED_MARGIN16, ST_SEEDED16, s);
    if (g_ev_start) (void)hipEventRecord(g_ev_start, s);
    knn_score_kernel<false><<<dim3((unsigned)(p.Tt_pad / FT), p.split), 256, SCORE_LDS, s>>>(
        w.s_bf16, (const unsigned short*)lib_bf16, M, p.tiles_total, p.tiles_per_split, p.P, w.cv, w.ci, nullptr, 0, 0, 0, nullptr, sa, 0);
    if (g_ev_stop) (void)hipEventRecord(g_ev_stop, s);
    rescore_launch((unsigned)((Tt + 3) / 4), s, w.cv, w.ci, p.P, KP, w.s_f32, rows_f32, norms, w.rows_hat, Tt, idx_base, k,
                                                               out_val, out_idx, nullptr, nullptr, 0, 0, w.list1, w.stats + ST_FLAG16,
                                                               CERT_Z, KH, 1.0f, SD_PRIOR16, w.det_q, w.det_lib, w.thr1, 0, w.lib_lo != nullptr ? SPLIT_BOUND : 0.0f);
    collect_tier_launch(w, lib_bf16, rows_f32, norms, M, Tt, idx_base, k, out_val, out_idx, s);
    ALIVE_CHECK_LAUNCH("alive_knn_search");
    return ALIVE_OK;
}

extern "C" int alive_knn_search(const float* src, int N, int T, const void* lib_bf16, const float* rows_f32,
                                const float* norms, int64_t M, int64_t idx_base, int k, float* out_val, int32_t* out_idx,
                                void* ws, void* stream) {
    return knn_search_impl(src, N, T, lib_bf16, rows_f32, norms, M, idx_base, k, out_val, out_idx, ws, stream, nullptr, nullptr);
}
extern "C" int alive_knn_search_strict(const float* src, int N, int T, const void* lib_bf16, const void* lib_lo, const float* rows_f32,
                                       const float* norms, const float* bound, int64_t M, int64_t idx_base, int k, float* out_val,
                                       int32_t* out_idx, void* ws, void* stream, void* ev_start, void* ev_stop) {
    ALIVE_CHECK_ARG(bound != nullptr, "alive_knn_search_strict: null bound (alive_library_rounding_bound)");
    return knn_search_impl(src, N, T, lib_bf16, rows_f32, norms, M, idx_base, k, out_val, out_idx, ws, stream,
                           (hipEvent_t)ev_start, (hipEvent_t)ev_stop, bound, lib_lo);
}

extern "C" int alive_library_pack_lo(const void* lib_bf16, const float* rows_f32, const float* norms, int64_t M, void* lib_lo,
                                     void* stream) {
    ALIVE_CHECK_ARG(lib_bf16 && rows_f32 && norms && lib_lo && M >= 1, "alive_library_pack_lo: bad args");
    const int64_t M_pad = alive_library_padded_rows(M);
    lib_lo_kernel<<<(unsigned)((M_pad * D + 255) / 256), 256, 0, (hipStream_t)stream>>>((const unsigned short*)lib_bf16, rows_f32, norms, M,
                                                                                     M_pad, (unsigned short*)lib_lo);
    ALIVE_CHECK_LAUNCH("alive_library_pack_lo");
    return ALIVE_OK;
}

extern "C" int alive_library_rounding_bound(const void* lib_bf16, const float* rows_f32, const float* norms, int64_t M,
                                            float* bound, void* stream) {
    ALIVE_CHECK_ARG(lib_bf16 && rows_f32 && norms && bound && M >= 1, "alive_library_rounding_bound: bad arguments");
    (void)hipMemsetAsync(bound, 0, sizeof(float), (hipStream_t)stream);
    lib_rounding_bound_kernel<<<(unsigned)((M + 3) / 4), 256, 0, (hipStream_t)stream>>>((const unsigned short*)lib_bf16, rows_f32, norms,
                                                                                        M, (unsigned*)bound);
    ALIVE_CHECK_LAUNCH("alive_library_rounding_bound");
    return ALIVE_OK;
}

extern "C" int alive_knn_search_timed(const float* src, int N, int T, const void* lib_bf16, const float* rows_f32,
                                      const float* norms, int64_t M, int64_t idx_base, int k, float* out_val, int32_t* out_idx,
                                      void* ws, void* stream, void* ev_start, void* ev_stop) {
    return knn_search_impl(src, N, T, lib_bf16, rows_f32, norms, M, idx_base, k, out_val, out_idx, ws, stream,
                           (hipEvent_t)ev_start, (hipEvent_t)ev_stop);
}

static int knn_search_fp8_impl(const float* src, int N, int T, const void* lib_f8, const void* lib_bf16, const float* rows_f32,
                               const float* norms, int64_t M, int64_t idx_base, int k, float* out_val, int32_t* out_idx,
                               void* ws, void* stream, hipEvent_t g_ev_start, hipEvent_t g_ev_stop, int fmt = 0,
                               const float* y_rot = nullptr, float rot_c0 = 0.0f, const float* y_sub = nullptr,
                               const void* lib_sub = nullptr, const float* rho = nullptr, const float* rows_hat = nullptr,
                               bool lazy_plain = false) {
    ALIVE_CHECK_ARG(src && lib_f8 && lib_bf16 && rows_f32 && norms && out_val && out_idx && ws, "alive_knn_search_fp8: null pointer");
    if (int rc = check_search_args("alive_knn_search_fp8", src, ws, N, T, k, M)) return rc;
    const int64_t Tt = (int64_t)N * T;
    if (k > KH)
        return knn_search_impl(src, N, T, lib_bf16, rows_f32, norms, M, idx_base, k, out_val, out_idx, ws, stream, g_ev_start, g_ev_stop);
    SearchWs w = ws_layout(ws, Tt, M, k, false, y_sub != nullptr);
    w.rows_hat = rows_hat;
    const bool lazy = lazy_plain && y_sub != nullptr;
    const bool f6 = fmt == 2;
    const SearchPlan& p = f6 ? w.p6 : w.p8;
    const SearchPlan& pp = f6 ? w.pp6 : w.pp;
    const int ft = f6 ? FT6 : FT, probe_pad = f6 ? w.probe_pad6 : w.probe_pad, lds = f6 ? SCORE6_LDS : SCORE8_LDS;
    const float pre = f6 ? 1.0f / (F6_SCALE * F6_SCALE) : 1.0f / (F8_SCALE * F8_SCALE),
                prior = f6 ? SD_PRIOR6 : (y_rot != nullptr ? SD_PRIOR8R : SD_PRIOR8);
    hipStream_t s = (hipStream_t)stream;
    if (Tt * k <= 64 && M <= SCAN_ROWS_MAX)
        return knn_scan_launch(src, T, Tt, rows_f32, norms, M, idx_base, k, w.s_f32, w.s_bf16, w.pv, w.pi, out_val, out_idx, w.stats, s, g_ev_start, g_ev_stop);
    if (int rc = lds_optin("alive_knn_search_fp8")) return rc;
    const int hist_tag = (int)(((uint64_t)M * 0x9E3779B1u) ^ ((uint64_t)Tt * 0x85EBCA77u) ^
                               (f6 ? (y_sub != nullptr ? 0x36u : 0x6u) : (y_rot != nullptr ? 0x18u : 0x8u))) | 1;
    stats_init_kernel<<<1, 64, 0, s>>>(w.stats, f6 ? TIER_FP6 : TIER_FP8, w.probe_n > 0 ? hist_tag : 0);
    src_prep_launch(w, src, T, Tt, s);
    if (f6) {
        const int64_t n32 = p.Tt_pad * D / 32;
        (void)hipMemsetAsync(w.clip6, 0, (size_t)p.Tt_pad, s);
        if (!lazy || w.probe_n > 0)
            to_fp6_kernel<<<(unsigned)((n32 + 255) / 256), 256, 0, s>>>(w.s_bf16, n32, w.p16.Tt_pad * D / 32, (u32x4*)w.s_f8, w.clip6, lazy ? 1 : 0,
                                                                        w.stats + ST_PROBE_GATE);
        if (y_sub != nullptr)
            sub_codes_kernel<<<(unsigned)(p.Tt_pad / 32), 256, 0, s>>>(y_sub, w.sub_nrm, T, Tt, p.Tt_pad, w.sub_f6, w.sub_g, w.sub_flag, w.stats);
    } else if (y_rot != nullptr) {
        rot_codes_kernel<<<(unsigned)(p.Tt_pad / 32), 256, 0, s>>>(y_rot, Tt, p.Tt_pad, T, 1, rot_c0, w.s_f8);
    } else {
        const int64_t n8 = p.Tt_pad * D / 8;
        src_to_fp8_kernel<<<(unsigned)((n8 + 255) / 256), 256, 0, s>>>(w.s_bf16, n8, (uint2*)w.s_f8);
    }
    int* mode = w.stats + ST_MODE;
    if (w.probe_n > 0) {
        const int* pgate = w.stats + ST_PROBE_GATE;
        probe_gather_kernel<<<(unsigned)probe_pad, 64, 0, s>>>(w.s_f8, Tt, w.probe_n, probe_pad, w.s_p8, w.p_list, pgate);
        if (f6)
            knn_probe6_kernel<<<dim3((unsigned)(probe_pad / ft), pp.split), 256, lds, s>>>(
                w.s_p8, (const unsigned char*)lib_f8, M, pp.tiles_total, pp.tiles_per_split, pp.P, w.cvp, w.cip, pgate);
        else
            knn_probe8_kernel<<<dim3((unsigned)(probe_pad / ft), pp.split), 256, lds, s>>>(
                w.s_p8, (const unsigned char*)lib_f8, M, pp.tiles_total, pp.tiles_per_split, pp.P, w.cvp, w.cip, pgate);
        rescore_launch((unsigned)((w.probe_n + 3) / 4), s, w.cvp, w.cip, pp.P, KP8, w.s_f32, rows_f32, norms, w.rows_hat, w.probe_n,
                                                                          idx_base, k, out_val, out_idx, w.p_list, pgate, GATE_BOOL, 0,
                                                                          w.p_list + probe_pad, w.stats + ST_PROBE_CNT, CERT_Z, KH8,
                                                                          pre, prior, nullptr, nullptr, nullptr, 0, 0.0f, f6 ? w.clip6 : nullptr);
        probe_decide_kernel<<<1, 1, 0, s>>>(w.stats, w.probe_n, PROBE_NUM, PROBE_DEN);
    }
    if (y_sub != nullptr) sub_select_kernel<<<(unsigned)((p.Tt_pad + 255) / 256), 256, 0, s>>>(w.sub_flag, w.clip6, p.Tt_pad, w.stats);
    if (lazy) {
        const int64_t n32 = p.Tt_pad * D / 32;
        to_fp6_kernel<<<(unsigned)((n32 + 255) / 256), 256, 0, s>>>(w.s_bf16, n32, w.p16.Tt_pad * D / 32, (u32x4*)w.s_f8, w.clip6, 2,
                                                                    w.probe_n > 0 ? w.stats + ST_PROBE_GATE : nullptr, w.stats + ST_SUB_GATE);
    }
    const SeedArgs sa8 = seeds_for(w, p.Tt_pad / ft, p.split, k, f6 ? SEED_MARGIN6 : SEED_MARGIN8, ST_SEEDED, s, f6 ? SEED_MIN_FB6 : SEED_MIN_FB);
    if (g_ev_start) (void)hipEventRecord(g_ev_start, s);
    if (y_sub != nullptr) {
        const int* gate = w.stats + ST_SUB_GATE;
        knn_sub6_kernel<<<dim3((unsigned)(p.Tt_pad / ft), p.split), 256, SUB6_LDS, s>>>(
            w.sub_f6, (const unsigned char*)lib_sub, rho, w.sub_g, M, p.tiles_total, p.tiles_per_split, p.P, w.cv, w.ci, gate, 0, 1, sa8);
        knn_score6_kernel<<<dim3((unsigned)(p.Tt_pad / ft), p.split), 256, lds, s>>>(
            w.s_f8, (const unsigned char*)lib_f8, M, p.tiles_total, p.tiles_per_split, p.P, w.cv, w.ci, gate, 1, 2, sa8);
    } else if (f6)
        knn_score6_kernel<<<dim3((unsigned)(p.Tt_pad / ft), p.split), 256, lds, s>>>(
            w.s_f8, (const unsigned char*)lib_f8, M, p.tiles_total, p.tiles_per_split, p.P, w.cv, w.ci, mode, -1, 0, sa8);
    else
        knn_score8_kernel<<<dim3((unsigned)(p.Tt_pad / ft), p.split), 256, lds, s>>>(
            w.s_f8, (const unsigned char*)lib_f8, M, p.tiles_total, p.tiles_per_split, p.P, w.cv, w.ci, mode, -1, 0, sa8);
    if (g_ev_stop) (void)hipEventRecord(g_ev_stop, s);
    rescore_launch((unsigned)((Tt + 3) / 4), s, w.cv, w.ci, p.P, KP8, w.s_f32, rows_f32, norms, w.rows_hat, Tt, idx_base, k,
                                                               out_val, out_idx, nullptr, mode, -1, 0, w.list0, w.stats + ST_FLAG8,
                                                               CERT_Z, KH8, pre, prior, nullptr, nullptr, nullptr, 0, 0.0f, f6 ? w.clip6 : nullptr);
    if (w.probe_n > 0) flag_all_kernel<<<(unsigned)((Tt + 255) / 256), 256, 0, s>>>(w.list0, w.stats + ST_FLAG8, Tt, mode, 0, 1);
    if (w.probe_n > 0) probe_history_kernel<<<1, 1, 0, s>>>(w.stats, Tt);
    bf16_tiers_launch(w, lib_bf16, rows_f32, norms, M, Tt, idx_base, k, out_val, out_idx, s);
    ALIVE_CHECK_LAUNCH("alive_knn_search_fp8");
    return ALIVE_OK;
}

extern "C" int alive_knn_search_fp8(const float* src, int N, int T, const void* lib_f8, const void* lib_bf16, const float* rows_f32,
                                    const float* norms, int64_t M, int64_t idx_base, int k, float* out_val, int32_t* out_idx,
                                    void* ws, void* stream) {
    return knn_search_fp8_impl(src, N, T, lib_f8, lib_bf16, rows_f32, norms, M, idx_base, k, out_val, out_idx, ws, stream, nullptr, nullptr);
}
extern "C" int alive_knn_search_fp8_timed(const float* src, int N, int T, const void* lib_f8, const void* lib_bf16, const float* rows_f32,
                                          const float* norms, int64_t M, int64_t idx_base, int k, float* out_val, int32_t* out_idx,
                                          void* ws, void* stream, void* ev_start, void* ev_stop) {
    return knn_search_fp8_impl(src, N, T, lib_f8, lib_bf16, rows_f32, norms, M, idx_base, k, out_val, out_idx, ws, stream,
                               (hipEvent_t)ev_start, (hipEvent_t)ev_stop);
}

extern "C" int alive_knn_rot_coordinates(void) { return ROT_C; }
extern "C" int alive_knn_rot_leading(void) { return ROT_A; }
extern "C" int alive_knn_rot_mixed(void) { return ROT_RHO; }
extern "C" int alive_library_pack_fp8_rot(const float* y_rows, int64_t m0, int64_t count, int64_t M, float c0, void* lib_f8, void* stream) {
    ALIVE_CHECK_ARG(y_rows && lib_f8 && M >= 1 && m0 >= 0 && count >= 1 && m0 + count <= M && (m0 % 32) == 0,
                    "alive_library_pack_fp8_rot: bad args (m0 must be a multiple of 32)");
    const int64_t m_pad = alive_library_padded_rows(M);
    const int64_t span = m0 + count == M ? m_pad - m0 : count;
    ALIVE_CHECK_ARG(span % 32 == 0, "alive_library_pack_fp8_rot: a chunk that is not the last must hold a multiple of 32 rows");
    rot_codes_kernel<<<(unsigned)(span / 32), 256, 0, (hipStream_t)stream>>>(y_rows, count, span, 0, 0, c0, (unsigned char*)lib_f8 + (size_t)m0 * D);
    ALIVE_CHECK_LAUNCH("alive_library_pack_fp8_rot");
    return ALIVE_OK;
}
extern "C" int alive_knn_search_fp8_rot_timed(const float* src, const float* y_rot, float c0, int N, int T, const void* lib_f8_rot, const void* lib_bf16,
                                              const float* rows_f32, const float* norms, int64_t M, int64_t idx_base, int k, float* out_val,
                                              int32_t* out_idx, void* ws, void* stream, void* ev_start, void* ev_stop) {
    ALIVE_CHECK_ARG(y_rot != nullptr, "alive_knn_search_fp8_rot: null rotated frames");
    return knn_search_fp8_impl(src, N, T, lib_f8_rot, lib_bf16, rows_f32, norms, M, idx_base, k, out_val, out_idx, ws, stream,
                               (hipEvent_t)ev_start, (hipEvent_t)ev_stop, 0, y_rot, c0);
}

extern "C" int alive_knn_search_fp6(const float* src, int N, int T, const void* lib_f6, const void* lib_bf16, const float* rows_f32,
                                    const float* norms, int64_t M, int64_t idx_base, int k, float* out_val, int32_t* out_idx,
                                    void* ws, void* stream) {
    return knn_search_fp8_impl(src, N, T, lib_f6, lib_bf16, rows_f32, norms, M, idx_base, k, out_val, out_idx, ws, stream, nullptr, nullptr, 2);
}
extern "C" int alive_knn_search_fp6_timed(const float* src, int N, int T, const void* lib_f6, const void* lib_bf16, const float* rows_f32,
                                          const float* norms, int64_t M, int64_t idx_base, int k, float* out_val, int32_t* out_idx,
                                          void* ws, void* stream, void* ev_start, void* ev_stop) {
    return knn_search_fp8_impl(src, N, T, lib_f6, lib_bf16, rows_f32, norms, M, idx_base, k, out_val, out_idx, ws, stream,
                               (hipEvent_t)ev_start, (hipEvent_t)ev_stop, 2);
}

extern "C" int alive_knn_search_fp6_sub_timed(const float* src, const float* y_sub, int N, int T, const void* lib_sub, const float* rho,
                                              const void* lib_f6, const void* lib_bf16, const float* rows_f32, const float* norms, int64_t M,
                                              int64_t idx_base, int k, float* out_val, int32_t* out_idx, void* ws, void* stream,
                                              void* ev_start, void* ev_stop) {
    ALIVE_CHECK_ARG(y_sub && lib_sub && rho, "alive_knn_search_fp6_sub: null subspace operand");
    return knn_search_fp8_impl(src, N, T, lib_f6, lib_bf16, rows_f32, norms, M, idx_base, k, out_val, out_idx, ws, stream,
                               (hipEvent_t)ev_start, (hipEvent_t)ev_stop, 2, nullptr, 0.0f, y_sub, lib_sub, rho);
}
extern "C" int alive_library_pack_unit_rows(const float* rows_f32, const float* norms, int64_t M, float* rows_hat, void* stream) {
    ALIVE_CHECK_ARG(rows_f32 && norms && rows_hat, "alive_library_pack_unit_rows: null pointer");
    ALIVE_CHECK_ARG(M >= 1 && M < (int64_t)1 << 31, "alive_library_pack_unit_rows: M out of range");
    const int64_t n4 = M * (D / 4);
    lib_unit_rows_kernel<<<(unsigned)((n4 + 255) / 256), 256, 0, (hipStream_t)stream>>>((const f32x4*)rows_f32, norms, n4, (f32x4*)rows_hat);
    ALIVE_CHECK_LAUNCH("alive_library_pack_unit_rows");
    return ALIVE_OK;
}

extern "C" int alive_knn_search_unit(const AliveKnnSearch* a, void* stream) {
    ALIVE_CHECK_ARG(a != nullptr, "alive_knn_search_unit: null arguments");
    hipEvent_t e0 = (hipEvent_t)a->ev_start, e1 = (hipEvent_t)a->ev_stop;
    switch (a->form) {
        case ALIVE_KNN_BF16:
            return knn_search_impl(a->src, a->N, a->T, a->lib_bf16, a->rows_f32, a->norms, a->M, a->idx_base, a->k, a->out_val, a->out_idx, a->ws,
                                   stream, e0, e1, nullptr, nullptr, a->rows_hat);
        case ALIVE_KNN_STRICT:
            ALIVE_CHECK_ARG(a->bound != nullptr, "alive_knn_search_unit: strict form without a bound (alive_library_rounding_bound)");
            return knn_search_impl(a->src, a->N, a->T, a->lib_bf16, a->rows_f32, a->norms, a->M, a->idx_base, a->k, a->out_val, a->out_idx, a->ws,
                                   stream, e0, e1, a->bound, a->lib_lo, a->rows_hat);
        case ALIVE_KNN_FP8:
        case ALIVE_KNN_FP6:
            return knn_search_fp8_impl(a->src, a->N, a->T, a->lib_stage, a->lib_bf16, a->rows_f32, a->norms, a->M, a->idx_base, a->k, a->out_val,
                                       a->out_idx, a->ws, stream, e0, e1, a->form == ALIVE_KNN_FP6 ? 2 : 0, nullptr, 0.0f, nullptr, nullptr,
                                       nullptr, a->rows_hat);
        case ALIVE_KNN_FP8_ROT:
            ALIVE_CHECK_ARG(a->y != nullptr, "alive_knn_search_unit: rotated form without the rotated frames");
            return knn_search_fp8_impl(a->src, a->N, a->T, a->lib_stage, a->lib_bf16, a->rows_f32, a->norms, a->M, a->idx_base, a->k, a->out_val,
                                       a->out_idx, a->ws, stream, e0, e1, 0, a->y, a->rot_c0, nullptr, nullptr, nullptr, a->rows_hat);
        case ALIVE_KNN_FP6_SUB: {
            ALIVE_CHECK_ARG((a->y || a->sub_w) && a->lib_sub && a->rho, "alive_knn_search_unit: null subspace operand");
            const float* y = a->y;
            const int64_t Tt = (int64_t)a->N * a->T;
            if (y == nullptr && a->src && a->ws && a->N > 0 && a->T > 0 && a->k >= 1 && a->k <= KH && !(Tt * a->k <= 64 && a->M <= SCAN_ROWS_MAX)) {
                ALIVE_CHECK_ARG(Tt * SUB_C < (1ll << 30), "alive_knn_search_unit: %lld frames exceed the plane GEMM's 32-bit offsets (pass y)", (long long)Tt);
                const SearchWs w = ws_layout(a->ws, Tt, a->M, a->k, false, true);
                if (int rc = alive_to_planes(a->src, a->N, D, a->T, 2, w.sub_planes, stream)) return rc;
                AliveGemm g{};
                g.W = a->sub_w; g.P = w.sub_planes; g.N = a->N; g.T = a->T; g.Ci = D; g.Co = SUB_C; g.planes = 2; g.Y = w.sub_y;
                if (int rc = alive_gemm_planes(&g, stream)) return rc;
                y = w.sub_y;
            }
            return knn_search_fp8_impl(a->src, a->N, a->T, a->lib_stage, a->lib_bf16, a->rows_f32, a->norms, a->M, a->idx_base, a->k, a->out_val,
                                       a->out_idx, a->ws, stream, e0, e1, 2, nullptr, 0.0f, y, a->lib_sub, a->rho, a->rows_hat, true);
        }
        default:
            ALIVE_CHECK_ARG(false, "alive_knn_search_unit: form %d", a->form);
    }
    return ALIVE_OK;
}
extern "C" int alive_knn_sub_coordinates(void) { return SUB_C; }
extern "C" size_t alive_library_fp6_sub_bytes(int64_t M) { return (size_t)alive_library_padded_rows(M) * SUB_K; }
extern "C" int alive_library_pack_fp6_sub(const float* y_rows, int64_t m0, int64_t count, int64_t M, void* lib_sub, float* rho, int* clip,
                                          void* stream) {
    ALIVE_CHECK_ARG(y_rows && lib_sub && rho && clip && M >= 1 && m0 >= 0 && count >= 1 && m0 + count <= M && (m0 % 32) == 0,
                    "alive_library_pack_fp6_sub: bad args (m0 must be a multiple of 32)");
    const int64_t m_pad = alive_library_padded_rows(M);
    const int64_t span = m0 + count == M ? m_pad - m0 : count;
    const int64_t n = span * (SUB_K / 32);
    lib_sub6_kernel<<<(unsigned)((n + 255) / 256), 256, 0, (hipStream_t)stream>>>(y_rows, count, span, (unsigned char*)lib_sub + (size_t)m0 * SUB_K,
                                                                                 rho + m0, clip);
    ALIVE_CHECK_LAUNCH("alive_library_pack_fp6_sub");
    return ALIVE_OK;
}

extern "C" const int* alive_knn_search_stats(int N, int T, int64_t M, void* ws) {
    return ws_layout(ws, (int64_t)N * T, M, 4).stats;
}

extern "C" int alive_debug_knn_stage_view(int64_t Tt, int64_t M, int k, int sub, int64_t* out, int n_out) {
    ALIVE_CHECK_ARG(out && n_out >= 25 && Tt >= 1 && M >= 1 && k >= 1 && k <= ALIVE_MAX_K, "alive_debug_knn_stage_view: bad args");
    const SearchWs w = ws_layout(nullptr, Tt, M, k, false, sub != 0);
    auto off = [](const void* p) { return p != nullptr ? (int64_t)(intptr_t)p : (int64_t)-1; };
    const int64_t head[8] = {off(w.s_bf16), off(w.s_f8), off(w.clip6), off(w.sub_f6), off(w.sub_g), off(w.cv), off(w.ci), (int64_t)w.bytes};
    for (int i = 0; i < 8; ++i) out[i] = head[i];
    const SearchPlan* plans[3] = {&w.p16, &w.p8, &w.p6};
    for (int i = 0; i < 3; ++i) {
        out[8 + 4 * i] = plans[i]->Tt_pad;
        out[9 + 4 * i] = plans[i]->tiles_total;
        out[10 + 4 * i] = plans[i]->tiles_per_split;
        out[11 + 4 * i] = plans[i]->P;
    }
    out[20] = KP; out[21] = KP8; out[22] = FT; out[23] = FT6; out[24] = LT;
    if (n_out >= 27) { out[25] = off(w.sub_planes); out[26] = off(w.sub_y); }
    return ALIVE_OK;
}

static int debug_rescore_check(const char* who, const AliveRescoreArgs* a, bool pool) {
    ALIVE_CHECK_ARG(a && a->cand_val && a->cand_idx && a->s_f32 && a->rows && a->norms && a->out_val && a->out_idx, "%s: null pointer", who);
    ALIVE_CHECK_ARG(a->k >= 1 && a->k <= KH, "%s: k=%d outside [1,%d]", who, a->k, KH);
    ALIVE_CHECK_ARG(a->P >= 1 && a->kp >= 1 && (int64_t)a->P * a->kp <= 1024, "%s: P=%d x kp=%d outside [1,1024] candidates", who, a->P, a->kp);
    ALIVE_CHECK_ARG(a->list_len == 8 || a->list_len == 16, "%s: list_len=%d is neither 8 nor 16", who, a->list_len);
    ALIVE_CHECK_ARG(a->M >= 1 && a->M < ((int64_t)1 << 31) && a->frames >= 1 && a->Tt >= 1 && a->Tt < ((int64_t)1 << 31),
                    "%s: M=%lld rows, %lld frames, Tt=%lld", who, (long long)a->M, (long long)a->frames, (long long)a->Tt);
    ALIVE_CHECK_ARG(a->frame_list != nullptr || a->Tt <= a->frames, "%s: Tt=%lld slots over %lld frames without a frame_list", who,
                    (long long)a->Tt, (long long)a->frames);
    const bool certify = a->flag_list != nullptr && a->collect == 0;
    ALIVE_CHECK_ARG((a->flag_list != nullptr) == (a->flag_cnt != nullptr), "%s: flag_list and flag_cnt go together", who);
    ALIVE_CHECK_ARG((a->collect == 0 || a->collect == 1) && (a->collect == 0 || a->flag_list != nullptr), "%s: collect=%d needs a flag_list", who, a->collect);
    ALIVE_CHECK_ARG(a->thr_list == nullptr || a->flag_list != nullptr, "%s: thr_list without a flag_list", who);
    ALIVE_CHECK_ARG(!certify || (a->P * a->kp) % a->list_len == 0, "%s: %d candidates are not whole lists of %d", who, a->P * a->kp, a->list_len);
    ALIVE_CHECK_ARG((a->det_q != nullptr) == (a->det_lib != nullptr), "%s: det_q and det_lib go together", who);
    ALIVE_CHECK_ARG(a->pre_scale > 0.0f && a->zsig >= 0.0f && a->sd_prior >= 0.0f && a->overflow_slack >= 0.0f, "%s: bad scale, z, prior or slack", who);
    if (a->gate_lo == GATE_BOOL) ALIVE_CHECK_ARG(a->gate_cnt != nullptr, "%s: an on / off gate without its word", who);
    else ALIVE_CHECK_ARG(a->gate_lo <= a->gate_hi, "%s: gate (%d, %d] is empty", who, a->gate_lo, a->gate_hi);
    if (pool) ALIVE_CHECK_ARG(certify && a->frame_list != nullptr && a->gate_lo != GATE_BOOL, "%s: the pool form certifies the slots of a plan", who);
    return ALIVE_OK;
}

extern "C" int alive_debug_knn_rescore(const AliveRescoreArgs* a, void* stream) {
    if (int rc = debug_rescore_check("alive_debug_knn_rescore", a, false)) return rc;
    rescore_launch((unsigned)((a->Tt + 3) / 4), (hipStream_t)stream, a->cand_val, a->cand_idx, a->P, a->kp, a->s_f32, a->rows, a->norms, nullptr, a->Tt,
                   a->idx_base, a->k, a->out_val, a->out_idx, a->frame_list, a->gate_cnt, a->gate_lo, a->gate_hi, a->flag_list, a->flag_cnt,
                   a->zsig, a->list_len, a->pre_scale, a->sd_prior, a->det_q, a->det_lib, a->thr_list, a->collect, a->overflow_slack,
                   a->force_fail);
    ALIVE_CHECK_LAUNCH("alive_debug_knn_rescore");
    return ALIVE_OK;
}


extern "C" int alive_debug_knn_pool_fields(int32_t* out, int n_out) {
    ALIVE_CHECK_ARG(out && n_out >= 4, "alive_debug_knn_pool_fields: bad args");
    out[0] = PG_FIELDS; out[1] = PG_VOICE; out[2] = PG_BLK0; out[3] = PG_K;
    return ALIVE_OK;
}

extern "C" int alive_knn_merge_gather(const float* cand_val, const int32_t* cand_idx, int n_shards, int k, double alpha,
                                      const float* rows_f32_full, const float* src, int N, int T, float* out,
                                      int32_t* final_idx, void* stream) {
    ALIVE_CHECK_ARG(cand_val && cand_idx && rows_f32_full && src && out, "alive_knn_merge_gather: null pointer");
    ALIVE_CHECK_ARG(k >= 1 && k <= ALIVE_MAX_K && n_shards >= 1 && n_shards * k <= 512,
                    "alive_knn_merge_gather: n_shards*k = %d exceeds 512", n_shards * k);
    ALIVE_CHECK_ARG(N > 0 && T > 0, "alive_knn_merge_gather: empty source");
    const int zs = (int64_t)cdiv(T, 32) * N < 64 ? D / 64 : 1;
    const dim3 g(cdiv(T, 32), N, zs);
    if (k <= 8 && n_shards * k <= 128)
        knn_merge_gather_kernel<2, 8><<<g, 256, 0, (hipStream_t)stream>>>(cand_val, cand_idx, n_shards, k, (float)alpha,
                                                                       (float)(1.0 - alpha), rows_f32_full, src, T, (int64_t)N * T, out, final_idx);
    else
        knn_merge_gather_kernel<8, ALIVE_MAX_K><<<g, 256, 0, (hipStream_t)stream>>>(cand_val, cand_idx, n_shards, k, (float)alpha,
                                                                                 (float)(1.0 - alpha), rows_f32_full, src, T, (int64_t)N * T, out, final_idx);
    ALIVE_CHECK_LAUNCH("alive_knn_merge_gather");
    return ALIVE_OK;
}

extern "C" int alive_dedup_pass(const float* val, const int32_t* idx, int64_t M, int k, double threshold, int32_t* state,
                                int32_t* undecided, void* stream) {
    ALIVE_CHECK_ARG(val && idx && state && undecided && M >= 1 && k >= 1, "alive_dedup_pass: bad arguments");
    dedup_pass_kernel<<<(unsigned)((M + 255) / 256), 256, 0, (hipStream_t)stream>>>(val, idx, M, k, (float)threshold, state, undecided);
    ALIVE_CHECK_LAUNCH("alive_dedup_pass");
    return ALIVE_OK;
}

extern "C" int alive_library_pack_rows(const float* tokens, int64_t M, int Dd, float* rows_f32, float* norms, void* stream) {
    ALIVE_CHECK_ARG(tokens && rows_f32 && norms, "alive_library_pack_rows: null pointer");
    ALIVE_CHECK_ARG(Dd == D, "alive_library_pack_rows: feature dim %d, expected %d", Dd, D);
    ALIVE_CHECK_ARG(M >= 1 && M < (int64_t)1 << 31, "alive_library_pack_rows: M out of range");
    const int64_t M_pad = alive_library_padded_rows(M);
    lib_pack_kernel<<<(unsigned)(M_pad / 64), 256, 0, (hipStream_t)stream>>>(tokens, M, M_pad, nullptr, rows_f32, norms);
    ALIVE_CHECK_LAUNCH("alive_library_pack_rows");
    return ALIVE_OK;
}

extern "C" size_t alive_knn_grouped_workspace_bytes(int N, int T, int k) {
    if (N < 1 || N > GR_MAX_ROWS || T < 1 || (int64_t)N * T > (int64_t)1 << 20 || k < 1 || k > KH) return 0;
    return grouped_ws_layout(nullptr, N, T, k).bytes;
}
// ... 333 lines not shown
```

### alive-vc_amd/module/_native.py

```python
import ctypes as C
import os

import torch

_HERE = os.path.dirname(os.path.abspath(__file__))
LIB_PATH = os.environ.get("ALIVE_VC_LIB", os.path.join(os.path.dirname(_HERE), "libalive_vc.so"))

_lib = None


class AliveConv(C.Structure):
    _fields_ = [
        ("W", C.c_void_p), ("bias", C.c_void_p), ("X", C.c_void_p),
        ("N", C.c_int), ("Ci", C.c_int), ("Tin", C.c_int), ("Co", C.c_int), ("K_pad", C.c_int),
        ("KW", C.c_int), ("stride", C.c_int), ("dil", C.c_int), ("pad_left", C.c_int), ("pad_mode", C.c_int),
        ("Tout", C.c_int), ("up", C.c_int), ("act", C.c_int),
        ("post_add", C.c_void_p), ("ch_scale", C.c_void_p), ("residual", C.c_void_p), ("skip", C.c_void_p),
        ("Y", C.c_void_p), ("Z", C.c_void_p), ("film", C.c_void_p),
        ("film_rows", C.c_int), ("Lf", C.c_int), ("film_scale_row", C.c_int), ("film_shift_row", C.c_int),
        ("precision", C.c_int), ("Ci_pad", C.c_int),
        ("film_t0", C.c_int), ("film_f0", C.c_int), ("film_ld", C.c_int),
        ("Xp", C.c_void_p), ("Zp", C.c_void_p), ("Yp", C.c_void_p), ("yp_planes", C.c_int),
    ]


class AliveGemm(C.Structure):
    _fields_ = [
        ("W", C.c_void_p), ("bias", C.c_void_p), ("P", C.c_void_p),
        ("N", C.c_int), ("T", C.c_int), ("Ci", C.c_int), ("Co", C.c_int), ("planes", C.c_int), ("act", C.c_int),
        ("post_add", C.c_void_p), ("ch_scale", C.c_void_p), ("residual", C.c_void_p),
        ("Y", C.c_void_p), ("Pout", C.c_void_p),
        ("b_plane", C.c_int64), ("b_win", C.c_int64), ("b_row", C.c_int), ("b_cblk", C.c_int), ("b_blk", C.c_int64),
        ("arg_val", C.c_void_p), ("arg_idx", C.c_void_p),
        ("Y2", C.c_void_p), ("y_split", C.c_int),
        ("f16s", C.c_int), ("wscale", C.c_void_p), ("in_unscale", C.c_float), ("pout_scale", C.c_float),
    ]


class AliveRescoreArgs(C.Structure):
    _fields_ = [
        ("cand_val", C.c_void_p), ("cand_idx", C.c_void_p), ("P", C.c_int), ("kp", C.c_int),
        ("s_f32", C.c_void_p), ("rows", C.c_void_p), ("norms", C.c_void_p),
        ("M", C.c_int64), ("frames", C.c_int64), ("Tt", C.c_int64), ("idx_base", C.c_int64), ("k", C.c_int),
        ("out_val", C.c_void_p), ("out_idx", C.c_void_p), ("frame_list", C.c_void_p), ("gate_cnt", C.c_void_p),
        ("gate_lo", C.c_int), ("gate_hi", C.c_int), ("flag_list", C.c_void_p), ("flag_cnt", C.c_void_p),
        ("zsig", C.c_float), ("list_len", C.c_int), ("pre_scale", C.c_float), ("sd_prior", C.c_float),
        ("det_q", C.c_void_p), ("det_lib", C.c_void_p), ("thr_list", C.c_void_p),
        ("collect", C.c_int), ("overflow_slack", C.c_float), ("force_fail", C.c_void_p),
    ]


class AliveKnnSearch(C.Structure):
    _fields_ = [
        ("form", C.c_int), ("N", C.c_int), ("T", C.c_int), ("k", C.c_int),
        ("src", C.c_void_p), ("lib_stage", C.c_void_p), ("lib_bf16", C.c_void_p), ("lib_lo", C.c_void_p),
        ("rows_f32", C.c_void_p), ("norms", C.c_void_p), ("rows_hat", C.c_void_p), ("bound", C.c_void_p),
        ("y", C.c_void_p), ("lib_sub", C.c_void_p), ("rho", C.c_void_p), ("sub_w", C.c_void_p), ("rot_c0", C.c_float),
        ("M", C.c_int64), ("idx_base", C.c_int64),
        ("out_val", C.c_void_p), ("out_idx", C.c_void_p), ("ws", C.c_void_p), ("ev_start", C.c_void_p), ("ev_stop", C.c_void_p),
    ]


KNN_BF16, KNN_STRICT, KNN_FP8, KNN_FP6, KNN_FP8_ROT, KNN_FP6_SUB = range(6)

_VP, _I, _I64, _F, _D, _SZ = C.c_void_p, C.c_int, C.c_int64, C.c_float, C.c_double, C.c_size_t

PROTOTYPES = {
    "alive_last_error": (C.c_char_p, []),
    "alive_version": (_I, []),
    "alive_library_padded_rows": (_I64, [_I64]),
    "alive_library_pack": (_I, [_VP, _I64, _I, _VP, _VP, _VP, _VP]),
    "alive_knn_workspace_bytes": (_SZ, [_I64, _I64]),
    "alive_knn_workspace_bytes_strict": (_SZ, [_I64, _I64]),
    "alive_knn_workspace_bytes_fast": (_SZ, [_I64, _I64]),
    "alive_knn_search": (_I, [_VP, _I, _I, _VP, _VP, _VP, _I64, _I64, _I, _VP, _VP, _VP, _VP]),
    "alive_library_fp8_bytes": (_SZ, [_I64]),
    "alive_library_rounding_bound": (_I, [_VP, _VP, _VP, _I64, _VP, _VP]),
    "alive_library_pack_lo": (_I, [_VP, _VP, _VP, _I64, _VP, _VP]),
    "alive_knn_search_strict": (_I, [_VP, _I, _I, _VP, _VP, _VP, _VP, _VP, _I64, _I64, _I, _VP, _VP, _VP, _VP, _VP, _VP]),
    "alive_library_pack_fp8": (_I, [_VP, _I64, _VP, _VP]),
    "alive_knn_search_fp8": (_I, [_VP, _I, _I, _VP, _VP, _VP, _VP, _I64, _I64, _I, _VP, _VP, _VP, _VP]),
    "alive_knn_search_stats": (_VP, [_I, _I, _I64, _VP]),
    "alive_debug_knn_stage_view": (_I, [_I64, _I64, _I, _I, _VP, _I]),
    "alive_debug_knn_rescore": (_I, [C.POINTER(AliveRescoreArgs), _VP]),
    "alive_debug_knn_rescore_pool": (_I, [C.POINTER(AliveRescoreArgs), _VP, _VP, _VP, _VP, _I, _VP]),
    "alive_debug_knn_pool_fields": (_I, [_VP, _I]),
    "alive_knn_search_timed": (_I, [_VP, _I, _I, _VP, _VP, _VP, _I64, _I64, _I, _VP, _VP, _VP, _VP, _VP, _VP]),
    "alive_knn_search_fp8_timed": (_I, [_VP, _I, _I, _VP, _VP, _VP, _VP, _I64, _I64, _I, _VP, _VP, _VP, _VP, _VP, _VP]),
    "alive_library_pack_fp6": (_I, [_VP, _I64, _VP, _VP]),
    "alive_knn_sub_coordinates": (_I, []),
    "alive_knn_workspace_bytes_sub": (_SZ, [_I64, _I64]),
    "alive_library_fp6_sub_bytes": (_SZ, [_I64]),
    "alive_library_pack_fp6_sub": (_I, [_VP, _I64, _I64, _I64, _VP, _VP, _VP, _VP]),
    "alive_knn_search_fp6_sub_timed": (_I, [_VP, _VP, _I, _I, _VP, _VP, _VP, _VP, _VP, _VP, _I64, _I64, _I, _VP, _VP, _VP, _VP, _VP, _VP]),
    "alive_library_pack_unit_rows": (_I, [_VP, _VP, _I64, _VP, _VP]),
    "alive_knn_search_unit": (_I, [C.POINTER(AliveKnnSearch), _VP]),
    "alive_knn_rot_coordinates": (_I, []),
    "alive_knn_rot_leading": (_I, []),
    "alive_knn_rot_mixed": (_I, []),
    "alive_library_pack_fp8_rot": (_I, [_VP, _I64, _I64, _I64, _F, _VP, _VP]),
    "alive_knn_search_fp8_rot_timed": (_I, [_VP, _VP, _F, _I, _I, _VP, _VP, _VP, _VP, _I64, _I64, _I, _VP, _VP, _VP, _VP, _VP, _VP]),
    "alive_knn_search_fp6": (_I, [_VP, _I, _I, _VP, _VP, _VP, _VP, _I64, _I64, _I, _VP, _VP, _VP, _VP]),
    "alive_knn_search_fp6_timed": (_I, [_VP, _I, _I, _VP, _VP, _VP, _VP, _I64, _I64, _I, _VP, _VP, _VP, _VP, _VP, _VP]),
    "alive_library_pack_rows": (_I, [_VP, _I64, _I, _VP, _VP, _VP]),
    "alive_knn_grouped_workspace_bytes": (_SZ, [_I, _I, _I]),
    "alive_knn_search_grouped": (_I, [_VP, _I, _I, _VP, _VP, _I64, _VP, _VP, _I, _VP, _VP, _VP, _VP]),
    "alive_knn_merge_gather_rows": (_I, [_VP, _VP, _I, _VP, _VP, _VP, _I, _I, _VP, _VP, _VP]),
    "alive_knn_blend_gather_rows": (_I, [_VP, _VP, _I, _VP, _VP, _VP, _VP, _VP, _I, _I, _VP, _VP]),
    "alive_knn_grouped_k_workspace_bytes": (_SZ, [_I, _I, _I]),
    "alive_knn_search_grouped_k": (_I, [_VP, _I, _I, _VP, _VP, _I64, _VP, _VP, _VP, _I, _VP, _VP, _VP, _VP]),
    "alive_knn_merge_gather_rows_k": (_I, [_VP, _VP, _VP, _I, _VP, _VP, _VP, _I, _I, _VP, _VP, _VP]),
    "alive_knn_blend_gather_rows_k": (_I, [_VP, _VP, _VP, _I, _VP, _VP, _VP, _VP, _VP, _I, _I, _VP, _VP]),
    "alive_pool_append": (_I, [_VP, _I64, _I64, _I64, _I, _VP, _VP, _I64, _I64, _VP, _VP]),
    "alive_pool_move_rows": (_I, [_VP, _VP, _I64, _I64, _I64, _I64, _VP]),
    "alive_pool_image_bytes": (_SZ, [_VP, _I, _VP]),
    "alive_pool_pack_images": (_I, [_VP, _VP, _I64, _VP, _VP, _I, _VP, _VP, _VP]),
    "alive_knn_pool_workspace_bytes": (_SZ, [_I, _I, _I, _I, _I64, _I64]),
    "alive_knn_search_pool": (_I, [_VP, _I, _I, _VP, _VP, _VP, _VP, _VP, _I64, _VP, _VP, _I, _I64, _VP, _I, _VP, _VP, _VP, _VP]),
    "alive_knn_pool_k_workspace_bytes": (_SZ, [_I, _I, _I, _I, _I64, _I64]),
    "alive_knn_search_pool_k": (_I, [_VP, _I, _I, _VP, _VP, _VP, _VP, _VP, _I64, _VP, _VP, _I, _I64, _VP, _VP, _I, _VP, _VP, _VP, _VP]),
    "alive_knn_pool_stats": (_VP, [_VP]),
    "alive_dedup_pass": (_I, [_VP, _VP, _I64, _I, _D, _VP, _VP, _VP]),
    "alive_knn_merge_gather": (_I, [_VP, _VP, _I, _I, _D, _VP, _VP, _I, _I, _VP, _VP, _VP]),
    "alive_conv1d": (_I, [C.POINTER(AliveConv), _VP]),
    "alive_conv1d_tiled": (_I, [C.POINTER(AliveConv), _VP]),
    "alive_conv_up_launches": (_I, [_I]),
    "alive_conv_up_min_blocks": (_I, [_I]),
    "alive_decoder_precision": (_I, [_I]),
    "alive_encoder_precision": (_I, [_I]),
    "alive_f16_saturations": (_I, [_I]),
    "alive_f16_saturations_clear": (_I, [_VP]),
    "alive_gelu_film": (_I, [_VP, _I, _I, _I, _VP, _I, _I, _I, _I, _I, _I, _I, _VP, _VP, _VP]),
    "alive_planes_bytes": (_SZ, [_I64, _I, _I]),
    "alive_to_planes": (_I, [_VP, _I, _I, _I, _I, _VP, _VP]),
    "alive_gemm_planes": (_I, [C.POINTER(AliveGemm), _VP]),
    "alive_argmax_merge": (_I, [_VP, _VP, _I, _I64, _VP, _VP]),
    "alive_filter_block_small_weights": (_I, [_I]),
    "alive_filter_block_small": (_I, [_VP, _I, _I, _I, _VP, _VP, _I, _I, _I, _VP, _VP, _VP]),
    "alive_filter_block_small_range": (_I, [_VP, _I, _I, _I, _VP, _VP, _I, _I, _I, _I, _I, _I, _VP, _VP, _VP]),
    "alive_filter_block_small_up_range": (_I, [_VP, _I, _I, _VP, _VP, _I, _I, _I, _I, _I, _I, _VP, _VP, _VP, _VP, _VP]),
    "alive_filter_block_small_wave_range": (_I, [_VP, _I, _I, _VP, _VP, _I, _I, _I, _I, _I, _I, _VP, _VP, _VP, _VP]),
    "alive_filter_block64_weights": (_I64, []),
    "alive_filter_block64": (_I, [_VP, _I, _I, _VP, _VP, _VP, _I, _I, _I, _VP, _VP, _VP]),
    "alive_filter_block64_range": (_I, [_VP, _I, _I, _VP, _VP, _VP, _I, _I, _I, _I, _I, _I, _VP, _VP, _VP]),
    "alive_filter_block64_range_fp16": (_I, [_VP, _I, _I, _VP, _VP, _VP, _I, _I, _I, _I, _I, _I, _VP, _VP, _VP]),
    "alive_filter_block256_workspace_bytes": (_I64, [_I, _I]),
    "alive_filter_block256_fp16": (_I, [_VP, _I, _I, _VP, _VP, _VP, _I, _I, _I, _I, _I, _I, _VP, _VP, _VP, _I64, _VP]),
    "alive_filter_block64s_workspace_bytes": (_I64, [_I, _I]),
    "alive_filter_block64s_fp16": (_I, [_VP, _I, _I, _VP, _VP, _VP, _I, _I, _I, _I, _I, _I, _VP, _VP, _VP, _I64, _VP]),
    "alive_filter_block64s_fp16_up": (_I, [_VP, _I, _I, _VP, _VP, _VP, _I, _I, _I, _I, _I, _I, _VP, _VP, _VP, _VP, _VP, _I64, _VP]),
    "alive_filter_source_in": (_I, [_VP, _I, _I, _VP, _VP, _VP, _VP, _VP, _VP]),
    "alive_filter_source_out": (_I, [_VP, _I, _I, _VP, _VP, _VP, _VP]),
    "alive_dwconv_norm": (_I, [_VP, _I, _I, _I, _VP, _VP, _I, _VP, _VP, _VP, _I, _I, _I, _F, _VP, _VP]),
    "alive_dwconv_norm_planes": (_I, [_VP, _I, _I, _I, _VP, _VP, _I, _VP, _VP, _VP, _I, _I, _I, _F, _I, _VP, _VP]),
    "alive_dwconv_norm_planes_f16s": (_I, [_VP, _I, _I, _I, _VP, _VP, _I, _VP, _VP, _VP, _I, _I, _I, _F, _F, _VP, _VP]),
    "alive_dwconv_norm_planes_ref": (_I, [_VP, _I, _I, _I, _VP, _VP, _I, _VP, _VP, _VP, _I, _I, _I, _F, _I, _VP, _VP, _F]),
    "alive_channel_norm": (_I, [_VP, _I, _I, _I, _VP, _VP, _F, _VP, _VP]),
    "alive_argmax_channels": (_I, [_VP, _I, _I, _I, _VP, _VP]),
    "alive_oscillator_workspace_bytes": (_SZ, [_I, _I, _I]),
    "alive_oscillator": (_I, [_VP, _VP, _VP, _I, _I, _I, _I, _F, _I, _I, _VP, _VP, _VP, _VP]),
    "alive_oscillator_range": (_I, [_VP, _VP, _VP, _I, _I, _I, _I, _F, _I, _I, _I, _I, _VP, _VP, _VP, _VP]),
    "alive_dft_basis_bytes": (_SZ, []),
    "alive_dft_basis": (_I, [_VP, _VP]),
    "alive_spectrogram_workspace_bytes": (_SZ, [_I, _I]),
    "alive_spectrogram": (_I, [_VP, _VP, _I, _I, _VP, _VP, _VP]),
    "alive_resample_taps": (_I, [_I, _I]),
    "alive_resample_length": (_I64, [_I64, _I, _I]),
    "alive_resample_filter": (_I, [_I, _I, _VP, _VP]),
    "alive_resample": (_I, [_VP, _I, _I, _I, _I, _VP, _F, _F, _VP, _I, _VP]),
    "alive_resample_rows": (_I, [_VP, _I, _I, _I, _I, _VP, _VP, _VP, _VP, _I, _VP]),
    "alive_resample_rows_multi": (_I, [_VP, _I, _I, _VP, _VP, _VP, _I, _VP, _I64, _I, _VP, _VP, _VP, _I, _VP, _VP]),
    "alive_pcm16_to_float": (_I, [_VP, _I64, _VP, _VP]),
    "alive_float_to_pcm16": (_I, [_VP, _I64, _VP, _VP]),
# ... 129 lines not shown
```

### alive-vc_amd/module/common.py

```python
import ctypes
import os
import weakref

import torch

from . import _native as nat

DIM = 768
DEFAULT_PREFILTER = "fp6"
_STAGES = ("bf16", "fp8", "fp6")


def _prefilter():
    return os.environ.get("ALIVE_KNN_PREFILTER", DEFAULT_PREFILTER)


def _rotate_allowed():
    return os.environ.get("ALIVE_KNN_ROTATE", "1") not in ("0", "false", "False")


ROT_MIN_LEAD = 0.10
ROT_MAX_TAIL = 1.0e-9


# ... 171 lines not shown
        val = torch.empty(n * t, k, dtype=torch.float32, device=source.device)
        idx = torch.empty(n * t, k, dtype=torch.int32, device=source.device)
        split = self.strict and self.lib_lo is not None
        sub = self.sub is not None and self.prefilter == "fp6" and not self.strict and self.rot is None
        wsb = L.alive_knn_workspace_bytes_strict if split else (L.alive_knn_workspace_bytes_sub if sub else L.alive_knn_workspace_bytes_fast)
        ws = self._ws.get(wsb(n * t, self.M), source.device)
        a = nat.AliveKnnSearch()
        a.N, a.T, a.k, a.M, a.idx_base = n, t, k, self.M, self.idx_base
        a.src, a.lib_bf16, a.rows_f32, a.norms = nat.ptr(source), nat.ptr(self.lib_bf16), nat.ptr(self.rows), nat.ptr(self.norms)
        a.rows_hat = nat.ptr(getattr(self, "rows_hat", None))
        a.out_val, a.out_idx, a.ws = nat.ptr(val), nat.ptr(idx), nat.ptr(ws)
        if events is not None:
            a.ev_start, a.ev_stop = events[0].cuda_event, events[1].cuda_event
        if self.strict:
            a.form, what = nat.KNN_STRICT, "alive_knn_search_strict"
            a.lib_lo, a.bound = nat.ptr(self.lib_lo), nat.ptr(self.bound)
        elif self.rot is not None:
            y = self._rotate_frames(source)
            a.form, what = nat.KNN_FP8_ROT, "alive_knn_search_fp8_rot"
            a.lib_stage, a.y, a.rot_c0 = nat.ptr(self.lib_f8), nat.ptr(y), self.rot["c0"]
        elif sub:
            a.form, what = nat.KNN_FP6_SUB, "alive_knn_search_fp6_sub"
            a.lib_stage, a.lib_sub, a.rho = nat.ptr(self.lib_f8), nat.ptr(self.sub["lib"]), nat.ptr(self.sub["rho"])
            if n * t * self.sub["co"] < 1 << 30:
                a.sub_w = nat.ptr(self.sub["W"])
            else:
                y = self._rotate_frames(source, self.sub)
                a.y = nat.ptr(y)
        elif self.lib_f8 is not None:
            a.form, what = (nat.KNN_FP6 if self.prefilter == "fp6" else nat.KNN_FP8), "alive_knn_search_" + self.prefilter
            a.lib_stage = nat.ptr(self.lib_f8)
        else:
            a.form, what = nat.KNN_BF16, "alive_knn_search"
        nat.check(L.alive_knn_search_unit(ctypes.byref(a), nat.stream()), what)
        self._last = (n, t, k, ws, sub)
        return val, idx


    def with_prefilter(self, prefilter, rotated=False):
        import copy
        if prefilter not in _STAGES:
            raise ValueError(prefilter)
        other = copy.copy(self)
        other.__dict__.pop("search", None)
        if rotated and self.rot is not None and prefilter == "fp8":
            other._ws, other._last = nat.Workspace(), None
            other.strict, other.bound, other.lib_lo, other.sub, other.sub_forms = False, None, None, None, []
            return other
        was_rot, other.rot = self.rot is not None, None
        other.sub = self.sub if prefilter == "fp6" else None
        other.sub_forms = self.sub_forms if prefilter == "fp6" else []
        other.fp6_declined = prefilter == "fp6" and self._fp6_would_clip()
        if other.fp6_declined:
            prefilter = "fp8"
        other.prefilter = prefilter
        other.strict, other.bound, other.lib_lo = False, None, None
        other._ws = nat.Workspace()
        other._last = None
        if prefilter == "bf16":
            other.lib_f8 = None
        elif self.lib_f8 is None or self.prefilter != prefilter or was_rot:
            other.lib_f8 = self._pack_stage(prefilter)
        return other

    def with_strict(self):
        other = self.with_prefilter("bf16")
        other.strict = True
        other._make_bound()
        return other

    def search_stats(self):
        last = getattr(self, "_last", None)
        if last is None:
            return None
        n, t, k, ws, sub = last
        torch.cuda.synchronize()
        st = {"prefilter": self.prefilter, "certificate": "deterministic" if self.strict else "statistical"}
        if getattr(self, "rot", None) is not None:
            st["rotated_operands"] = True
        off = nat.lib().alive_knn_search_stats(n, t, self.M, nat.ptr(ws)) - ws.data_ptr()
        c = ws[off:off + 128].view(torch.int32).tolist()
        tier = c[7]
        if sub and tier == 5:
            st.update(stage_form={1: "subspace", 2: "plain"}.get(c[21], "none"), frames_left_subspace=c[14] - c[15], frames_clipped=c[15])
        if tier == 1:
            return dict(st, tier="exact scan of every row (streaming)")
        if tier == 2:
            return dict(st, tier="exact scan of every row (k > 8)")
        if tier not in (3, 4, 5):
            raise RuntimeError(f"alive_knn_search_stats: no search has run on this workspace (tier word {tier})")
        few = 0
        if tier in (4, 5):
            few = c[0] if c[0] <= c[11] else 0
            st.update(frames_failed_fp8_certificate=c[0], frames_researched_on_bf16=0 if few else c[0], probe_sample=c[2],
                      probe_failed_fp8_certificate=c[3], probe_chose_bf16_first=bool(c[4]), fp8_blocks_seeded=c[9],
                      probe_skipped_on_history=bool(c[13]))
        direct = c[1] <= c[12]
        split = self.strict and getattr(self, "lib_lo", None) is not None
        st.update(bf16_blocks_seeded=c[10], frames_failed_bf16_certificate=c[1],
                  frames_collected_on_bf16=0 if direct or split else c[1],
                  frames_searched_exactly=few + (c[1] if direct else c[8]), frames=n * t)
        if split:
            st.update(frames_collected_on_split_bf16=0 if direct else c[1])
        return st

    def fallback_frames(self):
        st = self.search_stats()
        return 0 if st is None else int(st.get("frames_failed_fp8_certificate") or 0)


def merge_gather(cand_val, cand_idx, n_shards, k, alpha, rows_full, source, return_indices=False):
    n, d, t = source.shape
    out = torch.empty_like(source)
    fin = torch.empty(n * t, k, dtype=torch.int32, device=source.device) if return_indices else None
    nat.check(nat.lib().alive_knn_merge_gather(nat.ptr(cand_val), nat.ptr(cand_idx), n_shards, k, float(alpha),
                                               nat.ptr(rows_full), nat.ptr(source), n, t, nat.ptr(out), nat.ptr(fin),
                                               nat.stream()), "alive_knn_merge_gather")
    return (out, fin) if return_indices else out


_cache = {}


def _packed_for(reference_DxM):
    owner = reference_DxM._base if reference_DxM._base is not None else reference_DxM
    key = (reference_DxM.data_ptr(), tuple(reference_DxM.shape), tuple(reference_DxM.stride()), reference_DxM._version,
           str(reference_DxM.device), _prefilter(), _strict())
    hit = _cache.get(key)
    if hit is not None and hit[1]() is owner:
        return hit[0]
    if len(_cache) >= 4:
        _cache.pop(next(iter(_cache)))
    packed = PackedLibrary(reference_DxM)
    _cache[key] = (packed, weakref.ref(owner, lambda _r, key=key: _cache.pop(key, None)))
    return packed


def forget_packed():
    _cache.clear()


def match_features(source, reference, k=4, alpha=0.0, return_indices=False):
    if source.dim() != 3 or reference.dim() != 3 or source.shape[1] != DIM or reference.shape[1] != DIM:
        raise ValueError("match_features expects source [N,768,T] and reference [N,768,M]")
    if reference.shape[0] not in (1, source.shape[0]):
        raise ValueError("match_features: batch of reference must be 1 or equal to the batch of source")
    if reference.shape[2] < k:
        raise ValueError(f"match_features: library has {reference.shape[2]} vectors, fewer than k={k}")
    source = source.contiguous().float()
    if reference.shape[0] == 1:
        lib = _packed_for(reference[0])
        val, idx = lib.search(source, k)
        return merge_gather(val, idx, 1, k, alpha, lib.rows, source, return_indices)
    outs, idxs = [], []
    for n in range(source.shape[0]):
        lib = _packed_for(reference[n])
        s = source[n:n + 1].contiguous()
        val, idx = lib.search(s, k)
        r = merge_gather(val, idx, 1, k, alpha, lib.rows, s, return_indices)
        outs.append(r[0] if return_indices else r)
        if return_indices:
            idxs.append(r[1])
    out = torch.cat(outs, 0)
    return (out, torch.cat(idxs, 0)) if return_indices else out


_world_taps = {}
# ... 334 lines not shown
```

### include/alive_vc.h

```cpp
#ifndef ALIVE_VC_H
#define ALIVE_VC_H

#include <stddef.h>
#include <stdint.h>

#ifdef __cplusplus
extern "C" {
#endif

#define ALIVE_OK 0
#define ALIVE_ERR_ARG (-1)
#define ALIVE_ERR_LAUNCH (-2)

#define ALIVE_DIM 768
#define ALIVE_KPRIME 16
#define ALIVE_MAX_K 64

const char* alive_last_error(void);
int alive_version(void);

int64_t alive_library_padded_rows(int64_t M);
int alive_library_pack(const float* tokens_DxM, int64_t M, int D,
                       void* lib_bf16, float* rows_f32, float* norms, void* stream);

size_t alive_knn_workspace_bytes(int64_t Tt, int64_t M);
size_t alive_knn_workspace_bytes_strict(int64_t Tt, int64_t M);
size_t alive_knn_workspace_bytes_fast(int64_t Tt, int64_t M);
int alive_knn_search(const float* src, int N, int T,
                     const void* lib_bf16, const float* rows_f32, const float* norms,
                     int64_t M, int64_t idx_base, int k,
                     float* out_val, int32_t* out_idx, void* ws, void* stream);

int alive_library_rounding_bound(const void* lib_bf16, const float* rows_f32, const float* norms, int64_t M,
                                 float* bound, void* stream);
int alive_library_pack_lo(const void* lib_bf16, const float* rows_f32, const float* norms, int64_t M, void* lib_lo, void* stream);
int alive_knn_search_strict(const float* src, int N, int T,
                            const void* lib_bf16, const void* lib_lo, const float* rows_f32, const float* norms, const float* bound,
                            int64_t M, int64_t idx_base, int k,
                            float* out_val, int32_t* out_idx, void* ws, void* stream, void* ev_start, void* ev_stop);

size_t alive_library_fp8_bytes(int64_t M);
int alive_library_pack_fp8(const void* lib_bf16, int64_t M, void* lib_f8, void* stream);
int alive_knn_search_fp8(const float* src, int N, int T,
                         const void* lib_f8, const void* lib_bf16, const float* rows_f32, const float* norms,
                         int64_t M, int64_t idx_base, int k,
                         float* out_val, int32_t* out_idx, void* ws, void* stream);
const int* alive_knn_search_stats(int N, int T, int64_t M, void* ws);
int alive_debug_knn_stage_view(int64_t Tt, int64_t M, int k, int sub, int64_t* out, int n_out);

typedef struct AliveRescoreArgs {
    const float* cand_val;
    const int32_t* cand_idx;
    int P, kp;
    const float* s_f32;
    const float* rows;
    const float* norms;
    int64_t M, frames, Tt, idx_base;
    int k;
    float* out_val;
    int32_t* out_idx;
    const int32_t* frame_list;
    const int32_t* gate_cnt;
    int gate_lo, gate_hi;
    int32_t* flag_list;
    int32_t* flag_cnt;
    float zsig;
    int list_len;
    float pre_scale, sd_prior;
    const float* det_q;
    const float* det_lib;
    float* thr_list;
    int collect;
    float overflow_slack;
    const unsigned char* force_fail;
} AliveRescoreArgs;
int alive_debug_knn_rescore(const AliveRescoreArgs* a, void* stream);
int alive_debug_knn_rescore_pool(const AliveRescoreArgs* a, const int32_t* slot_grp, const int32_t* grp, int32_t* gfail, int32_t* fb,
                                 int groups, void* stream);
int alive_debug_knn_pool_fields(int32_t* out, int n_out);

int alive_knn_search_timed(const float* src, int N, int T,
                           const void* lib_bf16, const float* rows_f32, const float* norms,
                           int64_t M, int64_t idx_base, int k,
                           float* out_val, int32_t* out_idx, void* ws, void* stream, void* ev_start, void* ev_stop);
int alive_knn_search_fp8_timed(const float* src, int N, int T,
                               const void* lib_f8, const void* lib_bf16, const float* rows_f32, const float* norms,
                               int64_t M, int64_t idx_base, int k,
                               float* out_val, int32_t* out_idx, void* ws, void* stream, void* ev_start, void* ev_stop);

int alive_knn_rot_coordinates(void);
int alive_knn_rot_leading(void);
int alive_knn_rot_mixed(void);
int alive_library_pack_fp8_rot(const float* y_rows, int64_t m0, int64_t count, int64_t M, float c0, void* lib_f8, void* stream);
int alive_knn_search_fp8_rot_timed(const float* src, const float* y_rot, float c0, int N, int T,
                                   const void* lib_f8_rot, const void* lib_bf16, const float* rows_f32, const float* norms,
                                   int64_t M, int64_t idx_base, int k,
                                   float* out_val, int32_t* out_idx, void* ws, void* stream, void* ev_start, void* ev_stop);

int alive_library_pack_fp6(const void* lib_bf16, int64_t M, void* lib_f6, void* stream);
int alive_knn_search_fp6(const float* src, int N, int T,
                         const void* lib_f6, const void* lib_bf16, const float* rows_f32, const float* norms,
                         int64_t M, int64_t idx_base, int k,
                         float* out_val, int32_t* out_idx, void* ws, void* stream);
int alive_knn_search_fp6_timed(const float* src, int N, int T,
                               const void* lib_f6, const void* lib_bf16, const float* rows_f32, const float* norms,
                               int64_t M, int64_t idx_base, int k,
                               float* out_val, int32_t* out_idx, void* ws, void* stream, void* ev_start, void* ev_stop);

int alive_knn_sub_coordinates(void);
size_t alive_knn_workspace_bytes_sub(int64_t Tt, int64_t M);
size_t alive_library_fp6_sub_bytes(int64_t M);
int alive_library_pack_fp6_sub(const float* y_rows, int64_t m0, int64_t count, int64_t M, void* lib_sub, float* rho, int* clip,
                               void* stream);
int alive_knn_search_fp6_sub_timed(const float* src, const float* y_sub, int N, int T, const void* lib_sub, const float* rho,
                                   const void* lib_f6, const void* lib_bf16, const float* rows_f32, const float* norms, int64_t M,
                                   int64_t idx_base, int k, float* out_val, int32_t* out_idx, void* ws, void* stream,
                                   void* ev_start, void* ev_stop);

enum { ALIVE_KNN_BF16 = 0, ALIVE_KNN_STRICT = 1, ALIVE_KNN_FP8 = 2, ALIVE_KNN_FP6 = 3, ALIVE_KNN_FP8_ROT = 4, ALIVE_KNN_FP6_SUB = 5 };
typedef struct AliveKnnSearch {
    int form;
    int N, T, k;
    const float* src;
    const void* lib_stage;
    const void* lib_bf16;
    const void* lib_lo;
    const float* rows_f32;
    const float* norms;
    const float* rows_hat;
    const float* bound;
    const float* y;
    const void* lib_sub;
    const float* rho;
    const void* sub_w;
    float rot_c0;
    int64_t M, idx_base;
    float* out_val;
    int32_t* out_idx;
    void* ws;
    void* ev_start;
    void* ev_stop;
} AliveKnnSearch;
int alive_library_pack_unit_rows(const float* rows_f32, const float* norms, int64_t M, float* rows_hat, void* stream);
int alive_knn_search_unit(const AliveKnnSearch* a, void* stream);

int alive_knn_merge_gather(const float* cand_val, const int32_t* cand_idx, int n_shards, int k,
                           double alpha, const float* rows_f32_full, const float* src,
                           int N, int T, float* out, int32_t* final_idx, void* stream);

int alive_library_pack_rows(const float* tokens, int64_t M, int Dd, float* rows_f32, float* norms, void* stream);
size_t alive_knn_grouped_workspace_bytes(int N, int T, int k);
int alive_knn_search_grouped(const float* src, int N, int T, const float* rows_f32, const float* norms, int64_t P,
                             const int32_t* seg_lo, const int32_t* seg_len, int k, float* out_val, int32_t* out_idx,
                             void* ws, void* stream);
int alive_knn_merge_gather_rows(const float* cand_val, const int32_t* cand_idx, int k, const double* alpha,
                                const float* rows_f32_full, const float* src, int N, int T, float* out,
                                int32_t* final_idx, void* stream);
#define ALIVE_MAX_BLEND 4
int alive_knn_blend_gather_rows(const float* cand_val, const int32_t* cand_idx, int k, const int32_t* first,
                                const double* weight, const double* alpha, const float* rows_f32_full, const float* src,
                                int N, int T, float* out, void* stream);

size_t alive_knn_grouped_k_workspace_bytes(int N, int T, int k_max);
int alive_knn_search_grouped_k(const float* src, int N, int T, const float* rows_f32, const float* norms, int64_t P,
                               const int32_t* seg_lo, const int32_t* seg_len, const int32_t* k_row, int k_max, float* out_val,
                               int32_t* out_idx, void* ws, void* stream);
int alive_knn_merge_gather_rows_k(const float* cand_val, const int32_t* cand_idx, const int32_t* k_row, int k_max,
                                  const double* alpha, const float* rows_f32_full, const float* src, int N, int T, float* out,
                                  int32_t* final_idx, void* stream);
int alive_knn_blend_gather_rows_k(const float* cand_val, const int32_t* cand_idx, const int32_t* k_row, int k_max,
                                  const int32_t* first, const double* weight, const double* alpha, const float* rows_f32_full,
                                  const float* src, int N, int T, float* out, void* stream);

int alive_pool_append(const float* tokens, int64_t row_stride, int64_t col_stride, int64_t M, int Dd, float* rows_f32,
                      float* norms, int64_t capacity, int64_t at, int32_t* report, void* stream);
int alive_pool_move_rows(float* rows_f32, float* norms, int64_t capacity, int64_t src, int64_t dst, int64_t n, void* stream);

#define ALIVE_POOL_STATS 8
size_t alive_pool_image_bytes(const int32_t* seg_len, int V, int64_t* img_off);
int alive_pool_pack_images(const float* rows_f32, const float* norms, int64_t P, const int32_t* seg_lo, const int32_t* seg_len,
                           int V, void* images, float* bounds, void* stream);
size_t alive_knn_pool_workspace_bytes(int N, int T, int k, int V, int64_t P, int64_t max_len);
int alive_knn_search_pool(const float* src, int N, int T, const void* images, const int64_t* img_off, const float* rows_f32,
                          const float* norms, const float* bounds, int64_t P, const int32_t* seg_lo, const int32_t* seg_len,
                          int V, int64_t max_len, const int32_t* voice, int k, float* out_val, int32_t* out_idx, void* ws,
                          void* stream);
size_t alive_knn_pool_k_workspace_bytes(int N, int T, int k_max, int V, int64_t P, int64_t max_len);
int alive_knn_search_pool_k(const float* src, int N, int T, const void* images, const int64_t* img_off, const float* rows_f32,
                            const float* norms, const float* bounds, int64_t P, const int32_t* seg_lo, const int32_t* seg_len,
                            int V, int64_t max_len, const int32_t* voice, const int32_t* k_row, int k_max, float* out_val,
                            int32_t* out_idx, void* ws, void* stream);
const int* alive_knn_pool_stats(void* ws);
// ... 304 lines not shown
```

Before: 1.346 million.

## Add four-column-tile subspace kNN kernel with 16-bit tile-relative candidate indices

Adds a wide variant of the fp6 subspace scoring kernel that handles 512 frames per block (four 32-frame column tiles per wave) instead of three. Each streamed library tile is therefore reused across more query frames, which cuts library traffic per frame. To stay within LDS, candidate indices are stored as 16-bit tile offsets, and the full row index is rebuilt from the value's low bits at writeout. Two of the four query-operand sets are pinned to AGPRs to relieve register pressure. This adds a mode selector, changes padding, and resets seed flags whenever the grid sizes of the two stages differ.

Measured after the change: 1.362 million (median of 6 runs). 1.01x the previous value.

```diff
diff --git a/alive-vc_amd/csrc/knn.hip b/alive-vc_amd/csrc/knn.hip
--- a/alive-vc_amd/csrc/knn.hip
+++ b/alive-vc_amd/csrc/knn.hip
@@ -445,8 +445,8 @@
     return __builtin_amdgcn_readfirstlane(verdict[0]) != 0;
 }
 
-template <int KH_, int WF_ = 64, int FRAMES_ = 256>
-__device__ __forceinline__ void seeds_publish(const SeedArgs& sa, const float* Lv, const int* Li, int64_t frame0, int split, bool seeded) {
+template <int KH_, int WF_ = 64, int FRAMES_ = 256, typename LI = int>
+__device__ __forceinline__ void seeds_publish(const SeedArgs& sa, const float* Lv, const LI* Li, int64_t frame0, int split, bool seeded) {
     constexpr int LW_ = 4 * 2 * WF_;
     for (int col = threadIdx.x; col < FRAMES_; col += 256) {
         const int lcb = (col / WF_) * (2 * WF_) + ((col % WF_) >> 5) * 64 + (col & 31);
@@ -456,7 +456,9 @@
             for (int e = 0; e < 2 * KH_; ++e) {
                 const int o = (e % KH_) * LW_ + lcb + (e / KH_) * 32;
                 const float v = Lv[o];
-                if (Li[o] >= 0 && v < prev) m = fmaxf(m, v);
+                bool real;
+                if constexpr (sizeof(LI) == 2) real = Li[o] != (LI)0xFFFF; else real = Li[o] >= 0;
+                if (real && v < prev) m = fmaxf(m, v);
             }
             prev = m;
         }
@@ -898,6 +900,8 @@
     extern __shared__ __attribute__((aligned(16))) unsigned char smem[];
     float* Lv = (float*)(smem + 2 * ABUF_);
     int* Li = (int*)(Lv + FT8 * KP8);
+    constexpr bool WIDE = NCT8 == 4;
+    unsigned short* Lt = (unsigned short*)(Lv + FT8 * KP8);
 
     const int tid = threadIdx.x, lane = tid & 63;
     const int w = __builtin_amdgcn_readfirstlane(tid >> 6);
@@ -922,7 +926,11 @@
 #pragma unroll
     for (int ni = 0; ni < NCT8; ++ni)
 #pragma unroll
-        for (int q = 0; q < KH8; ++q) { Lv[q * LW8 + w * (2 * WF8) + ni * 64 + lane] = seed[ni]; Li[q * LW8 + w * (2 * WF8) + ni * 64 + lane] = -1; }
+        for (int q = 0; q < KH8; ++q) {
+            Lv[q * LW8 + w * (2 * WF8) + ni * 64 + lane] = seed[ni];
+            if constexpr (WIDE) Lt[q * LW8 + w * (2 * WF8) + ni * 64 + lane] = 0xFFFFu;
+            else Li[q * LW8 + w * (2 * WF8) + ni * 64 + lane] = -1;
+        }
 
     const int dma_row = 8 * w + (lane >> 3);
     const int dma_chunk = (lane & 7) ^ (lane >> 3);
@@ -936,6 +944,7 @@
     if (tile_begin < tile_end) issue_tile(tile_begin, 0);
 
     v8i bq[NCT8][NK];
+    constexpr int WIDE_AGPR_NI = 2;
 #pragma unroll
     for (int ni = 0; ni < NCT8; ++ni) {
         const unsigned char* fp = s_f8 + (size_t)(frame0 + WF8 * w + 32 * ni + lr) * KD + 32 * lh;
@@ -944,7 +953,14 @@
             if constexpr (FMT == 2) {
                 const u32x4 lo = *(const u32x4*)(fp + 64 * ks);
                 const uint2 hi = *(const uint2*)(fp + 64 * ks + 16);
-                bq[ni][ks] = v8i{(int)lo[0], (int)lo[1], (int)lo[2], (int)lo[3], (int)hi.x, (int)hi.y, 0, 0};
+                if constexpr (NCT8 == 4) {
+                    typedef int v6i __attribute__((ext_vector_type(6)));
+                    v6i t = {(int)lo[0], (int)lo[1], (int)lo[2], (int)lo[3], (int)hi.x, (int)hi.y};
+                    if (ni >= WIDE_AGPR_NI) asm volatile("" : "+a"(t));
+                    bq[ni][ks] = v8i{t[0], t[1], t[2], t[3], t[4], t[5], 0, 0};
+                } else {
+                    bq[ni][ks] = v8i{(int)lo[0], (int)lo[1], (int)lo[2], (int)lo[3], (int)hi.x, (int)hi.y, 0, 0};
+                }
             } else {
                 const u32x4 lo = *(const u32x4*)(fp + 64 * ks), hi = *(const u32x4*)(fp + 64 * ks + 16);
                 bq[ni][ks] = v8i{(int)lo[0], (int)lo[1], (int)lo[2], (int)lo[3], (int)hi[0], (int)hi[1], (int)hi[2], (int)hi[3]};
@@ -1032,7 +1048,8 @@
             const int tq = tpos >> 2;
             if (has) {
                 lv[tpos * LW8] = mx;
-                li[tpos * LW8] = (int)(row0 + ((__float_as_uint(mx) & 3u) + 8u * ((__float_as_uint(mx) >> 2) & 3u)) + 4 * lh);
+                if constexpr (WIDE) Lt[lc0 + ni * 64 + tpos * LW8] = (unsigned short)(tile - tile_begin);
+                else li[tpos * LW8] = (int)(row0 + ((__float_as_uint(mx) & 3u) + 8u * ((__float_as_uint(mx) >> 2) & 3u)) + 4 * lh);
             }
             const float* qb = lv + (tq * 4) * LW8;
             const float x0 = qb[0], x1 = qb[LW8], x2 = qb[2 * LW8], x3 = qb[3 * LW8];
@@ -1087,7 +1104,8 @@
         if (has) {
             const unsigned u = __float_as_uint(m1);
             lv[tpos * LW8] = m1;
-            li[tpos * LW8] = (int)(row0 + ((u & 3u) + 8u * ((u >> 2) & 3u)) + 4 * lh);
+            if constexpr (WIDE) Lt[lc0 + ni * 64 + tpos * LW8] = (unsigned short)(tile - tile_begin);
+            else li[tpos * LW8] = (int)(row0 + ((u & 3u) + 8u * ((u >> 2) & 3u)) + 4 * lh);
         }
         x0 = (has && te == 0) ? m1 : x0;
         x1 = (has && te == 1) ? m1 : x1;
@@ -1199,6 +1217,100 @@
             fold_now3(A0, A1, A2, tile, RA);
         } else if (tile_begin < tile_end) {
             fold_now3(B0, B1, B2, tile_end - 1, RB);
+        }
+    }
+    } else if constexpr (NCT8 == 4) {
+    static_assert(NK == 8 && FMT == 2, "the four-tile form exists for the subspace stage");
+    auto do_tile4 = [&](int tile, f32x16& c0, f32x16& c1, f32x16& c2, f32x16& c3, f32x16& p0, f32x16& p1, f32x16& p2, f32x16& p3,
+                        float* rv, float* rn) {
+        const int buf = (tile - tile_begin) & 1;
+        const int next_tile = tile + 1 < tile_end ? tile + 1 : tile;
+        const unsigned char* gnext = lib + ((size_t)next_tile * LT + dma_row) * KD + dma_chunk * 16;
+        unsigned char* lnext = smem + (buf ^ 1) * ABUF_ + w * PIECE;
+        const unsigned char* Ab = smem + buf * ABUF_;
+#pragma unroll
+        for (int r = 0; r < 16; ++r) { c0[r] = 0.0f; c1[r] = 0.0f; c2[r] = 0.0f; c3[r] = 0.0f; }
+        load_rho(tile, rn);
+        v8i a[2];
+        a[0] = load_a(Ab, 0);
+        float pm0 = -INFINITY, pm1 = -INFINITY, pm2 = -INFINITY, pm3 = -INFINITY;
+        ALIVE_CHAIN_GAP(7);
+#define K8_STEP4(ks, AFTER0, AFTER1, AFTER2, AFTER3)                                                                             \
+        {                                                                                                                        \
+            __builtin_amdgcn_sched_barrier(0);                                                                                   \
+            c0 = __builtin_amdgcn_mfma_scale_f32_32x32x64_f8f6f4(a[(ks) & 1], bq[0][ks], c0, FMT, FMT, 0, 127, 0, 127);          \
+            __builtin_amdgcn_sched_barrier(0);                                                                                   \
+            if ((ks) + 1 < NK) a[((ks) + 1) & 1] = load_a(Ab, (ks) + 1);                                                         \
+            if ((ks) < NSEG)                                                                                                     \
+                __builtin_amdgcn_global_load_lds((gptr_t)(gnext + (ks) * 128), (lptr_t)(lnext + (ks) * 4 * PIECE), 16, 0, 0);    \
+            AFTER0;                                                                                                              \
+            __builtin_amdgcn_sched_barrier(0);                                                                                   \
+            c1 = __builtin_amdgcn_mfma_scale_f32_32x32x64_f8f6f4(a[(ks) & 1], bq[1][ks], c1, FMT, FMT, 0, 127, 0, 127);          \
+            __builtin_amdgcn_sched_barrier(0);                                                                                   \
+            AFTER1;                                                                                                              \
+            __builtin_amdgcn_sched_barrier(0);                                                                                   \
+            c2 = __builtin_amdgcn_mfma_scale_f32_32x32x64_f8f6f4(a[(ks) & 1], bq[2][ks], c2, FMT, FMT, 0, 127, 0, 127);          \
+            __builtin_amdgcn_sched_barrier(0);                                                                                   \
+            AFTER2;                                                                                                              \
+            __builtin_amdgcn_sched_barrier(0);                                                                                   \
+            c3 = __builtin_amdgcn_mfma_scale_f32_32x32x64_f8f6f4(a[(ks) & 1], bq[3][ks], c3, FMT, FMT, 0, 127, 0, 127);          \
+            __builtin_amdgcn_sched_barrier(0);                                                                                   \
+            AFTER3;                                                                                                              \
+        }
+        f32x16 v0, v1, v2, v3;
+        auto acc_read = [&](const f32x16& a_, int lo, int hi, f32x16& v) {
+#pragma unroll
+            for (int r = lo; r < hi; ++r) asm volatile("v_accvgpr_read_b32 %0, %1" : "=v"(v[r]) : "a"(a_[r]));
+        };
+        auto acc_pin = [&]() { asm volatile("" : "+a"(c0), "+a"(c1), "+a"(c2), "+a"(c3)); };
+        auto acc_pin2 = [&]() { asm volatile("" : "+a"(c0), "+a"(c1)); };
+        auto acc_pin3 = [&]() { asm volatile("" : "+a"(c0), "+a"(c1), "+a"(c2)); };
+        K8_STEP4(0, (void)0, (acc_pin2(), acc_read(p0, 0, 8, v0)), (acc_pin3(), acc_read(p0, 8, 16, v0), mask_ragged(v0, tile - 1)),
+                 (acc_pin(), pm0 = max8g(v0, 0, pm0, 0, rv)))
+        K8_STEP4(1, (void)0, pm0 = max8g(v0, 8, pm0, 0, rv), fold_rare(v0, 0, tile - 1, pm0), (acc_pin(), acc_read(p1, 0, 8, v1)))
+        K8_STEP4(2, (void)0, (acc_pin(), acc_read(p1, 8, 16, v1), mask_ragged(v1, tile - 1)), (acc_pin(), pm1 = max8g(v1, 0, pm1, 1, rv)),
+                 pm1 = max8g(v1, 8, pm1, 1, rv))
+        K8_STEP4(3, (void)0, fold_rare(v1, 1, tile - 1, pm1), (acc_pin(), acc_read(p2, 0, 8, v2)),
+                 (acc_pin(), acc_read(p2, 8, 16, v2), mask_ragged(v2, tile - 1)))
+        K8_STEP4(4, (acc_pin(), pm2 = max8g(v2, 0, pm2, 2, rv)), pm2 = max8g(v2, 8, pm2, 2, rv), fold_rare(v2, 2, tile - 1, pm2),
+                 (acc_pin(), acc_read(p3, 0, 8, v3)))
+        K8_STEP4(5, (acc_pin(), acc_read(p3, 8, 16, v3), mask_ragged(v3, tile - 1)), (acc_pin(), pm3 = max8g(v3, 0, pm3, 3, rv)),
+                 pm3 = max8g(v3, 8, pm3, 3, rv), fold_rare(v3, 3, tile - 1, pm3))
+        K8_STEP4(6, (void)0, (void)0, (void)0, (void)0)
+        K8_STEP4(7, (void)0, (void)0, (void)0, (void)0)
+#undef K8_STEP4
+        acc_pin();
+        __syncthreads();
+    };
+    auto fold_now4 = [&](f32x16& p0, f32x16& p1, f32x16& p2, f32x16& p3, int tile, float* rv) {
+        mask_ragged(p0, tile);
+        mask_ragged(p1, tile);
+        mask_ragged(p2, tile);
+        mask_ragged(p3, tile);
+        (void)max8g(p0, 0, max8g(p0, 8, -INFINITY, 0, rv), 0, rv);
+        (void)max8g(p1, 0, max8g(p1, 8, -INFINITY, 1, rv), 1, rv);
+        (void)max8g(p2, 0, max8g(p2, 8, -INFINITY, 2, rv), 2, rv);
+        (void)max8g(p3, 0, max8g(p3, 8, -INFINITY, 3, rv), 3, rv);
+        fold_rare(p0, 0, tile, max8(p0, 8, max8(p0, 0, -INFINITY)));
+        fold_rare(p1, 1, tile, max8(p1, 8, max8(p1, 0, -INFINITY)));
+        fold_rare(p2, 2, tile, max8(p2, 8, max8(p2, 0, -INFINITY)));
+        fold_rare(p3, 3, tile, max8(p3, 8, max8(p3, 0, -INFINITY)));
+    };
+    {
+        f32x16 A0, A1, A2, A3, B0, B1, B2, B3;
+        float RA[16], RB[16];
+#pragma unroll
+        for (int r = 0; r < 16; ++r) { B0[r] = -INFINITY; B1[r] = -INFINITY; B2[r] = -INFINITY; B3[r] = -INFINITY; RA[r] = 0.0f; RB[r] = 0.0f; }
+        int tile = tile_begin;
+        for (; tile + 1 < tile_end; tile += 2) {
+            do_tile4(tile, A0, A1, A2, A3, B0, B1, B2, B3, RB, RA);
+            do_tile4(tile + 1, B0, B1, B2, B3, A0, A1, A2, A3, RA, RB);
+        }
+        if (tile < tile_end) {
+            do_tile4(tile, A0, A1, A2, A3, B0, B1, B2, B3, RB, RA);
+            fold_now4(A0, A1, A2, A3, tile, RA);
+        } else if (tile_begin < tile_end) {
+            fold_now4(B0, B1, B2, B3, tile_end - 1, RB);
         }
     }
     } else {
@@ -1278,9 +1390,18 @@
         const int lc = (col / WF8) * (2 * WF8) + ((col % WF8) >> 5) * 64 + (k / KH8) * 32 + (col & 31);
         const size_t o = (((size_t)(frame0 + col)) * P + split) * KP8 + k;
         cand_val[o] = Lv[(k % KH8) * LW8 + lc];
-        cand_idx[o] = Li[(k % KH8) * LW8 + lc];
-    }
-    if (sa.tau != nullptr) seeds_publish<KH8, WF8, FT8>(sa, Lv, Li, frame0, split, seeded);
+        if constexpr (WIDE) {
+            const unsigned t = Lt[(k % KH8) * LW8 + lc], u = __float_as_uint(Lv[(k % KH8) * LW8 + lc]);
+            cand_idx[o] = t == 0xFFFFu ? -1 : (int)((tile_begin + (int)t) * LT + (u & 3u) + 8u * ((u >> 2) & 3u) + 4 * (k / KH8));
+        } else {
+            cand_idx[o] = Li[(k % KH8) * LW8 + lc];
+        }
+    }
+    if constexpr (WIDE) {
+        if (sa.tau != nullptr) seeds_publish<KH8, WF8, FT8>(sa, Lv, Lt, frame0, split, seeded);
+    } else {
+        if (sa.tau != nullptr) seeds_publish<KH8, WF8, FT8>(sa, Lv, Li, frame0, split, seeded);
+    }
 }
 
 __global__ __launch_bounds__(256, 1) void knn_score8_kernel(const unsigned char* __restrict__ s_f8, const unsigned char* __restrict__ lib,
@@ -1314,6 +1435,18 @@
                                                           float* __restrict__ cand_val, int* __restrict__ cand_idx,
                                                           const int* __restrict__ gate_cnt, int gate_lo, int gate_hi, SeedArgs sa) {
     knn_score8_body<2, 3, NK_SUB>(s_sub, lib_sub, M, tiles_total, tiles_per_split, P, cand_val, cand_idx, gate_cnt, gate_lo, gate_hi, sa,
+                                  rho, gq);
+}
+constexpr int FT6W = 4 * 32 * 4;
+constexpr int SUB6W_LDS = 2 * 4 * (SUB_K / 128) * PIECE + FT6W * KP8 * 6;
+constexpr int SUB6W_MAX_TILES = 65535;
+static_assert(SUB6W_LDS == SUB6_LDS && SUB6W_LDS <= 163840, "the wide subspace kernel's LDS");
+__global__ __launch_bounds__(256, 1) void knn_sub6w_kernel(const unsigned char* __restrict__ s_sub, const unsigned char* __restrict__ lib_sub,
+                                                           const float* __restrict__ rho, const float* __restrict__ gq,
+                                                           int64_t M, int tiles_total, int tiles_per_split, int P,
+                                                           float* __restrict__ cand_val, int* __restrict__ cand_idx,
+                                                           const int* __restrict__ gate_cnt, int gate_lo, int gate_hi, SeedArgs sa) {
+    knn_score8_body<2, 4, NK_SUB>(s_sub, lib_sub, M, tiles_total, tiles_per_split, P, cand_val, cand_idx, gate_cnt, gate_lo, gate_hi, sa,
                                   rho, gq);
 }
 
@@ -2377,6 +2510,7 @@
 enum { ST_FLAG8 = 0, ST_FLAG16 = 1, ST_PROBE_N = 2, ST_PROBE_FAIL = 3, ST_MODE = 4, ST_FIRST = 5, ST_PROBE_CNT = 6, ST_TIER = 7, ST_FLAGC = 8, ST_SEEDED = 9, ST_SEEDED16 = 10, ST_RESEARCH_MIN = 11, ST_COLLECT_MIN = 12,
        ST_PROBE_SKIPPED = 13,
        ST_SUB_FLAG = 14, ST_SUB_CLIP = 15, ST_SUB_FORM = 20, ST_SUB_GATE = 21,
+       ST_SUB_FRAMES = 22,
        ST_HIST_TAG = 16, ST_HIST_STREAK = 17, ST_HIST_CALLS = 18, ST_PROBE_GATE = 19,
        ST_WORDS = 32 };
 constexpr int PROBE_EVERY = 16, PROBE_STREAK = 2;
@@ -2461,12 +2595,13 @@
     }
 }
 __global__ __launch_bounds__(256) void sub_select_kernel(const unsigned char* __restrict__ flag, unsigned char* __restrict__ clip6,
-                                                         int64_t n, int* __restrict__ stats) {
+                                                         int64_t n, int* __restrict__ stats, int stage_frames) {
     const bool sub = stats[ST_SUB_FLAG] <= RESEARCH_MIN;
     const int64_t i = (int64_t)blockIdx.x * 256 + threadIdx.x;
     if (sub && i < n && flag[i] != 0) clip6[i] = 1;
     if (i == 0) {
         stats[ST_SUB_FORM] = sub ? 1 : 2;
+        stats[ST_SUB_FRAMES] = stage_frames;
         stats[ST_SUB_GATE] = stats[ST_MODE] != 0 ? 0 : (sub ? 1 : 2);
     }
 }
@@ -2594,6 +2729,7 @@
 struct SearchWs {
     SearchPlan p16, p8, pt, pp;
     SearchPlan p6, pp6;
+    SearchPlan p6w;
     SearchPlan pa;
     int fcap, probe_n, probe_pad, probe_pad6;
     float* s_f32; unsigned short* s_bf16; unsigned char* s_f8;
@@ -2624,8 +2760,9 @@
     w.p16 = make_plan(Tt, M);
     w.p8 = make_plan(Tt, M, MAX_SPLIT8);
     w.p6 = make_plan(Tt, M, MAX_SPLIT8, FT6);
+    w.p6w = make_plan(Tt, M, MAX_SPLIT8, FT6W);
     const int64_t Tp = w.p16.Tt_pad;
-    const int64_t Tp8 = w.p6.Tt_pad > Tp ? w.p6.Tt_pad : Tp;
+    const int64_t Tp8 = std::max(std::max(w.p6.Tt_pad, w.p6w.Tt_pad), Tp);
     w.fcap = Tp < FCAP ? (int)Tp : FCAP;
     w.pt = make_plan(w.fcap < FPLAN ? w.fcap : FPLAN, M);
     w.pa = make_plan(FT, M);
@@ -2639,7 +2776,7 @@
     w.s_f32 = a.take<float>((size_t)Tt * D);
     w.s_bf16 = a.take<unsigned short>((size_t)Tp * D);
     w.s_f8 = a.take<unsigned char>((size_t)Tp8 * D);
-    const size_t c8a = (size_t)Tp * w.p8.P * KP8, c8b = (size_t)w.p6.Tt_pad * w.p6.P * KP8;
+    const size_t c8a = (size_t)Tp * w.p8.P * KP8, c8b = (size_t)Tp8 * std::max(w.p6.P, w.p6w.P) * KP8;
     const size_t c16 = (size_t)Tp * w.p16.P * KP, c8 = c8a > c8b ? c8a : c8b;
     w.cv = a.take<float>(c16 > c8 ? c16 : c8);
     w.ci = a.take<int>(c16 > c8 ? c16 : c8);
@@ -2670,7 +2807,7 @@
     w.rows_b = (int)(c2n / (size_t)Tp < 1024 ? c2n / (size_t)Tp : 1024);
     w.lib_lo = nullptr;
     w.tau = a.take<float>((size_t)Tp8);
-    w.tau_flag = a.take<int>((size_t)(Tp / FT) * (MAX_SPLIT > MAX_SPLIT8 ? MAX_SPLIT : MAX_SPLIT8));
+    w.tau_flag = a.take<int>((size_t)(Tp8 / FT) * (MAX_SPLIT > MAX_SPLIT8 ? MAX_SPLIT : MAX_SPLIT8));
     w.det_q = nullptr;
     w.det_lib = nullptr;
     w.rows_hat = nullptr;
@@ -3056,13 +3193,33 @@
     return ALIVE_OK;
 }
 
+static int g_sub_frames = -1;
+static int sub_frames_mode() {
+    if (g_sub_frames < 0) {
+        const char* e = getenv("ALIVE_KNN_SUB_FRAMES");
+        const int v = e != nullptr ? atoi(e) : 0;
+        g_sub_frames = v == FT6 || v == FT6W ? v : 0;
+    }
+    return g_sub_frames;
+}
+extern "C" int alive_knn_sub_frames(int mode) {
+    if (mode == FT6 || mode == FT6W) g_sub_frames = mode;
+    else if (mode < 0) g_sub_frames = 0;
+    return sub_frames_mode();
+}
+static bool sub_wide(const SearchPlan& pw) {
+    const int mode = sub_frames_mode();
+    if (mode == FT6 || pw.tiles_per_split > SUB6W_MAX_TILES) return false;
+    return mode == FT6W || pw.Tt_pad / FT6W >= SEED_MIN_FB6;
+}
+
 static int lds_optin(const char* what) {
     static LdsOptIn optin8, optin6, optin16, optin_split, optin_sub;
     hipError_t e = optin8.ensure({(const void*)knn_score8_kernel, (const void*)knn_probe8_kernel}, SCORE8_LDS);
     if (e == hipSuccess) e = optin6.ensure({(const void*)knn_score6_kernel, (const void*)knn_probe6_kernel}, SCORE6_LDS);
     if (e == hipSuccess) e = optin16.ensure({(const void*)knn_score_kernel<false>, (const void*)knn_score_kernel<true>}, SCORE_LDS);
     if (e == hipSuccess) e = optin_split.ensure({(const void*)knn_collect_split_kernel}, SPLIT_LDS);
-    if (e == hipSuccess) e = optin_sub.ensure({(const void*)knn_sub6_kernel}, SUB6_LDS);
+    if (e == hipSuccess) e = optin_sub.ensure({(const void*)knn_sub6_kernel, (const void*)knn_sub6w_kernel}, SUB6_LDS);
     if (e != hipSuccess) {
         alive_set_error("%s: cannot reserve %d B of LDS: %s", what, SCORE_LDS, hipGetErrorString(e));
         return ALIVE_ERR_LAUNCH;
@@ -3271,8 +3428,10 @@
     w.rows_hat = rows_hat;
     const bool lazy = lazy_plain && y_sub != nullptr;
     const bool f6 = fmt == 2;
-    const SearchPlan& p = f6 ? w.p6 : w.p8;
+    const bool wide = f6 && y_sub != nullptr && sub_wide(w.p6w);
+    const SearchPlan& p = f6 ? (wide ? w.p6w : w.p6) : w.p8;
     const SearchPlan& pp = f6 ? w.pp6 : w.pp;
+    const int64_t Tpad = wide ? std::max(w.p6.Tt_pad, w.p6w.Tt_pad) : p.Tt_pad;
     const int ft = f6 ? FT6 : FT, probe_pad = f6 ? w.probe_pad6 : w.probe_pad, lds = f6 ? SCORE6_LDS : SCORE8_LDS;
     const float pre = f6 ? 1.0f / (F6_SCALE * F6_SCALE) : 1.0f / (F8_SCALE * F8_SCALE),
                 prior = f6 ? SD_PRIOR6 : (y_rot != nullptr ? SD_PRIOR8R : SD_PRIOR8);
@@ -3285,13 +3444,13 @@
     stats_init_kernel<<<1, 64, 0, s>>>(w.stats, f6 ? TIER_FP6 : TIER_FP8, w.probe_n > 0 ? hist_tag : 0);
     src_prep_launch(w, src, T, Tt, s);
     if (f6) {
-        const int64_t n32 = p.Tt_pad * D / 32;
-        (void)hipMemsetAsync(w.clip6, 0, (size_t)p.Tt_pad, s);
+        const int64_t n32 = Tpad * D / 32;
+        (void)hipMemsetAsync(w.clip6, 0, (size_t)Tpad, s);
         if (!lazy || w.probe_n > 0)
             to_fp6_kernel<<<(unsigned)((n32 + 255) / 256), 256, 0, s>>>(w.s_bf16, n32, w.p16.Tt_pad * D / 32, (u32x4*)w.s_f8, w.clip6, lazy ? 1 : 0,
                                                                         w.stats + ST_PROBE_GATE);
         if (y_sub != nullptr)
-            sub_codes_kernel<<<(unsigned)(p.Tt_pad / 32), 256, 0, s>>>(y_sub, w.sub_nrm, T, Tt, p.Tt_pad, w.sub_f6, w.sub_g, w.sub_flag, w.stats);
+            sub_codes_kernel<<<(unsigned)(Tpad / 32), 256, 0, s>>>(y_sub, w.sub_nrm, T, Tt, Tpad, w.sub_f6, w.sub_g, w.sub_flag, w.stats);
     } else if (y_rot != nullptr) {
         rot_codes_kernel<<<(unsigned)(p.Tt_pad / 32), 256, 0, s>>>(y_rot, Tt, p.Tt_pad, T, 1, rot_c0, w.s_f8);
     } else {
@@ -3314,19 +3473,27 @@
                                                                           pre, prior, nullptr, nullptr, nullptr, 0, 0.0f, f6 ? w.clip6 : nullptr);
         probe_decide_kernel<<<1, 1, 0, s>>>(w.stats, w.probe_n, PROBE_NUM, PROBE_DEN);
     }
-    if (y_sub != nullptr) sub_select_kernel<<<(unsigned)((p.Tt_pad + 255) / 256), 256, 0, s>>>(w.sub_flag, w.clip6, p.Tt_pad, w.stats);
+    if (y_sub != nullptr)
+        sub_select_kernel<<<(unsigned)((Tpad + 255) / 256), 256, 0, s>>>(w.sub_flag, w.clip6, Tpad, w.stats, wide ? FT6W : FT6);
     if (lazy) {
-        const int64_t n32 = p.Tt_pad * D / 32;
+        const int64_t n32 = Tpad * D / 32;
         to_fp6_kernel<<<(unsigned)((n32 + 255) / 256), 256, 0, s>>>(w.s_bf16, n32, w.p16.Tt_pad * D / 32, (u32x4*)w.s_f8, w.clip6, 2,
                                                                     w.probe_n > 0 ? w.stats + ST_PROBE_GATE : nullptr, w.stats + ST_SUB_GATE);
     }
-    const SeedArgs sa8 = seeds_for(w, p.Tt_pad / ft, p.split, k, f6 ? SEED_MARGIN6 : SEED_MARGIN8, ST_SEEDED, s, f6 ? SEED_MIN_FB6 : SEED_MIN_FB);
+    const int64_t fb = wide ? p.Tt_pad / FT6W : p.Tt_pad / ft, fb6 = w.p6.Tt_pad / FT6;
+    const SeedArgs sa8 = seeds_for(w, fb, p.split, k, f6 ? SEED_MARGIN6 : SEED_MARGIN8, ST_SEEDED, s, f6 ? SEED_MIN_FB6 : SEED_MIN_FB);
+    if (wide && sa8.flag != nullptr && fb6 > fb)
+        (void)hipMemsetAsync(w.tau_flag, 0, (size_t)fb6 * p.split * sizeof(int), s);
     if (g_ev_start) (void)hipEventRecord(g_ev_start, s);
     if (y_sub != nullptr) {
         const int* gate = w.stats + ST_SUB_GATE;
-        knn_sub6_kernel<<<dim3((unsigned)(p.Tt_pad / ft), p.split), 256, SUB6_LDS, s>>>(
-            w.sub_f6, (const unsigned char*)lib_sub, rho, w.sub_g, M, p.tiles_total, p.tiles_per_split, p.P, w.cv, w.ci, gate, 0, 1, sa8);
-        knn_score6_kernel<<<dim3((unsigned)(p.Tt_pad / ft), p.split), 256, lds, s>>>(
+        if (wide)
+            knn_sub6w_kernel<<<dim3((unsigned)fb, p.split), 256, SUB6W_LDS, s>>>(
+                w.sub_f6, (const unsigned char*)lib_sub, rho, w.sub_g, M, p.tiles_total, p.tiles_per_split, p.P, w.cv, w.ci, gate, 0, 1, sa8);
+        else
+            knn_sub6_kernel<<<dim3((unsigned)fb, p.split), 256, SUB6_LDS, s>>>(
+                w.sub_f6, (const unsigned char*)lib_sub, rho, w.sub_g, M, p.tiles_total, p.tiles_per_split, p.P, w.cv, w.ci, gate, 0, 1, sa8);
+        knn_score6_kernel<<<dim3((unsigned)fb6, p.split), 256, lds, s>>>(
             w.s_f8, (const unsigned char*)lib_f8, M, p.tiles_total, p.tiles_per_split, p.P, w.cv, w.ci, gate, 1, 2, sa8);
     } else if (f6)
         knn_score6_kernel<<<dim3((unsigned)(p.Tt_pad / ft), p.split), 256, lds, s>>>(
@@ -3482,6 +3649,37 @@
     }
     out[20] = KP; out[21] = KP8; out[22] = FT; out[23] = FT6; out[24] = LT;
     if (n_out >= 27) { out[25] = off(w.sub_planes); out[26] = off(w.sub_y); }
+    if (n_out >= 32) {
+        out[27] = w.p6w.Tt_pad; out[28] = w.p6w.tiles_total; out[29] = w.p6w.tiles_per_split; out[30] = w.p6w.P; out[31] = FT6W;
+    }
+    return ALIVE_OK;
+}
+
+extern "C" int alive_debug_knn_sub_stage(const void* s_sub, const float* g, int64_t Tt_pad, const void* lib_sub, const float* rho, int64_t M,
+                                         int split, float* cand_val, int32_t* cand_idx, int* frames_out, void* stream) {
+    ALIVE_CHECK_ARG(s_sub && g && lib_sub && rho && cand_val && cand_idx && frames_out, "alive_debug_knn_sub_stage: null pointer");
+    ALIVE_CHECK_ARG(Tt_pad >= 1 && Tt_pad % (3 * FT6W) == 0 && Tt_pad < ((int64_t)1 << 24), "alive_debug_knn_sub_stage: Tt_pad must be a multiple of %d", 3 * FT6W);
+    ALIVE_CHECK_ARG(M >= 1 && M < ((int64_t)1 << 31) - TILE && split >= 1 && split <= MAX_SPLIT8, "alive_debug_knn_sub_stage: M or split out of range");
+    if (int rc = lds_optin("alive_debug_knn_sub_stage")) return rc;
+    SearchPlan p;
+    p.Tt = p.Tt_pad = Tt_pad;
+    p.tiles_total = (int)(((M + TILE - 1) / TILE * TILE) / LT);
+    p.split = p.P = split;
+    p.tiles_per_split = (p.tiles_total + split - 1) / split;
+    const int mode = sub_frames_mode();
+    const bool wide = mode != FT6 && p.tiles_per_split <= SUB6W_MAX_TILES;
+    const SeedArgs none{nullptr, nullptr, 0, 0.0f, nullptr};
+    hipStream_t s = (hipStream_t)stream;
+    if (wide)
+        knn_sub6w_kernel<<<dim3((unsigned)(Tt_pad / FT6W), split), 256, SUB6W_LDS, s>>>(
+            (const unsigned char*)s_sub, (const unsigned char*)lib_sub, rho, g, M, p.tiles_total, p.tiles_per_split, p.P, cand_val, cand_idx,
+            nullptr, 0, 1, none);
+    else
+        knn_sub6_kernel<<<dim3((unsigned)(Tt_pad / FT6), split), 256, SUB6_LDS, s>>>(
+            (const unsigned char*)s_sub, (const unsigned char*)lib_sub, rho, g, M, p.tiles_total, p.tiles_per_split, p.P, cand_val, cand_idx,
+            nullptr, 0, 1, none);
+    ALIVE_CHECK_LAUNCH("alive_debug_knn_sub_stage");
+    *frames_out = wide ? FT6W : FT6;
     return ALIVE_OK;
 }
 
diff --git a/alive-vc_amd/module/_native.py b/alive-vc_amd/module/_native.py
--- a/alive-vc_amd/module/_native.py
+++ b/alive-vc_amd/module/_native.py
@@ -82,6 +82,7 @@
     "alive_knn_search_fp8": (_I, [_VP, _I, _I, _VP, _VP, _VP, _VP, _I64, _I64, _I, _VP, _VP, _VP, _VP]),
     "alive_knn_search_stats": (_VP, [_I, _I, _I64, _VP]),
     "alive_debug_knn_stage_view": (_I, [_I64, _I64, _I, _I, _VP, _I]),
+    "alive_debug_knn_sub_stage": (_I, [_VP, _VP, _I64, _VP, _VP, _I64, _I, _VP, _VP, _VP, _VP]),
     "alive_debug_knn_rescore": (_I, [C.POINTER(AliveRescoreArgs), _VP]),
     "alive_debug_knn_rescore_pool": (_I, [C.POINTER(AliveRescoreArgs), _VP, _VP, _VP, _VP, _I, _VP]),
     "alive_debug_knn_pool_fields": (_I, [_VP, _I]),
@@ -89,6 +90,7 @@
     "alive_knn_search_fp8_timed": (_I, [_VP, _I, _I, _VP, _VP, _VP, _VP, _I64, _I64, _I, _VP, _VP, _VP, _VP, _VP, _VP]),
     "alive_library_pack_fp6": (_I, [_VP, _I64, _VP, _VP]),
     "alive_knn_sub_coordinates": (_I, []),
+    "alive_knn_sub_frames": (_I, [_I]),
     "alive_knn_workspace_bytes_sub": (_SZ, [_I64, _I64]),
     "alive_library_fp6_sub_bytes": (_SZ, [_I64]),
     "alive_library_pack_fp6_sub": (_I, [_VP, _I64, _I64, _I64, _VP, _VP, _VP, _VP]),
diff --git a/alive-vc_amd/module/common.py b/alive-vc_amd/module/common.py
--- a/alive-vc_amd/module/common.py
+++ b/alive-vc_amd/module/common.py
@@ -277,7 +277,8 @@
         c = ws[off:off + 128].view(torch.int32).tolist()
         tier = c[7]
         if sub and tier == 5:
-            st.update(stage_form={1: "subspace", 2: "plain"}.get(c[21], "none"), frames_left_subspace=c[14] - c[15], frames_clipped=c[15])
+            st.update(stage_form={1: "subspace", 2: "plain"}.get(c[21], "none"), frames_left_subspace=c[14] - c[15], frames_clipped=c[15],
+                      stage_frames=c[22])
         if tier == 1:
             return dict(st, tier="exact scan of every row (streaming)")
         if tier == 2:
diff --git a/include/alive_vc.h b/include/alive_vc.h
--- a/include/alive_vc.h
+++ b/include/alive_vc.h
@@ -47,6 +47,8 @@
                          float* out_val, int32_t* out_idx, void* ws, void* stream);
 const int* alive_knn_search_stats(int N, int T, int64_t M, void* ws);
 int alive_debug_knn_stage_view(int64_t Tt, int64_t M, int k, int sub, int64_t* out, int n_out);
+int alive_debug_knn_sub_stage(const void* s_sub, const float* g, int64_t Tt_pad, const void* lib_sub, const float* rho, int64_t M, int split,
+                              float* cand_val, int32_t* cand_idx, int* frames_out, void* stream);
 
 typedef struct AliveRescoreArgs {
     const float* cand_val;
@@ -108,6 +110,7 @@
                                float* out_val, int32_t* out_idx, void* ws, void* stream, void* ev_start, void* ev_stop);
 
 int alive_knn_sub_coordinates(void);
+int alive_knn_sub_frames(int mode);
 size_t alive_knn_workspace_bytes_sub(int64_t Tt, int64_t M);
 size_t alive_library_fp6_sub_bytes(int64_t M);
 int alive_library_pack_fp6_sub(const float* y_rows, int64_t m0, int64_t count, int64_t M, void* lib_sub, float* rho, int* clip,
```
